# google-research/snap

Hardware: AMD Instinct MI355X
Metric: localization_scenes_per_sec (higher is better)
Workload: dtype f32 (tensors, accumulation, every non-GEMM op); conv / dense products on the bf16 matrix cores: operands split into 2 bf16 parts, 3 part products per MAC, ~2^-17 per product; 1 GPU; C2: 8 scenes/GPU, 4 StreetView views @512px + aerial, 128x128x60 voxel BEV @0.2m, ResNet-50 encoders, 10001 pose hypotheses; scenes_per_gpu=8, batches_in_flight=2, global_batch=8, parallelism=scene-sharded x1, no data-path collective, mode=inference forward (BEVLocalizer.apply, train=False)

## Files before the change

### include/snap_hip.h

```cpp
#ifndef SNAP_HIP_H_
#define SNAP_HIP_H_

#include <stddef.h>
#include <stdint.h>

#ifdef __cplusplus
extern "C" {
#endif

typedef enum SnapStatus {
  SNAP_OK = 0,
  SNAP_ERR_BAD_SHAPE = -1,
  SNAP_ERR_UNSUPPORTED = -2,
  SNAP_ERR_NULL = -3,
  SNAP_ERR_LAUNCH = -4,
  SNAP_ERR_WORKSPACE = -5
} SnapStatus;

#define SNAP_ABI_VERSION 29
int snap_abi_version(void);
const char* snap_status_string(int status);
const char* snap_build_arch(void);

enum { SNAP_PRO_NONE = 0, SNAP_PRO_AFFINE = 1, SNAP_PRO_GN_RELU = 2,
       SNAP_PRO_RELU_GN = 3, SNAP_PRO_RELU = 4 };
enum { SNAP_EPI_BIAS = 1, SNAP_EPI_RELU = 2, SNAP_EPI_RESIDUAL = 4,
       SNAP_EPI_UPSAMPLE2X_ADD = 8, SNAP_EPI_ROWMASK = 16,
       SNAP_EPI_GELU = 32  };

typedef struct SnapConvDesc {
  int32_t N, H, W, Cin, Cin_stride;
  int32_t KH, KW, stride, pad_t, pad_l;
  int32_t Ho, Wo, Cout, Cout_stride;
  int32_t prologue;
  int32_t epilogue;
  float in_scale, in_shift;
  int32_t tile_hint;
} SnapConvDesc;

int snap_conv2d_nhwc_f32(const SnapConvDesc* desc, const float* x, const float* w,
                         float* y, const float* gn_mu, const float* gn_sc,
                         const float* gn_beta, const float* bias,
                         const float* residual, const float* up_prev,
                         const uint8_t* row_mask, void* stream);

typedef struct SnapConvExtras {
  const int32_t* rows_in;
  const int32_t* rows_out;
  const int32_t* row_count;
  float* gn_partial;
  size_t gn_partial_bytes;
  int32_t gn_partial_relu;
  void* workspace;
  size_t workspace_bytes;
  const void* w_bf16;
  size_t w_bf16_bytes;
  int32_t w_split_parts;
  int32_t w_split_root;
  float* gn_partial2;
  size_t gn_partial2_bytes;
  int32_t gn_partial2_done;
  int32_t x_presplit;
  int32_t ps_tile;
  int32_t ps_res_init;
  int32_t bk_hint;
  int32_t tune_flags;
  int32_t gn_partial_rows;
  int32_t w_half;
  int32_t x_half;
  void* y_half;
  const float* gnb_x;
  const float* gnb_mu;
  const float* gnb_rstd;
  const float* gnb_gamma;
  const float* gnb_beta;
  int32_t gnb_mode;
} SnapConvExtras;
#define SNAP_TUNE_NO_HALO 1
#define SNAP_TUNE_NO_PLAIN 8
#define SNAP_TUNE_RS_NSPLIT_SHIFT 4
int32_t snap_conv2d_presplit_tile_rows(const SnapConvDesc* desc, int32_t ps_tile);
size_t snap_conv2d_presplit_gn_partial_bytes(const SnapConvDesc* desc, int32_t ps_tile);
size_t snap_conv2d_presplit_workspace_bytes(const SnapConvDesc* desc, int32_t ps_tile);
int32_t snap_conv2d_presplit_supported(const SnapConvDesc* desc);
int snap_gn_norm_split_f32(const float* y, const float* partial, int32_t N, int32_t HW, int32_t C,
                           int32_t groups, float eps, int32_t tile_rows, const float* gamma,
                           const float* beta, void* out, float* mu, float* sc, void* stream);
int snap_presplit_f32(const float* x, int64_t rows, int32_t C, void* out, void* stream);

int snap_conv2d_nhwc_ex_f32(const SnapConvDesc* desc, const float* x, const float* w,
                            float* y, const float* gn_mu, const float* gn_sc,
                            const float* gn_beta, const float* bias,
                            const float* residual, const float* up_prev,
                            const uint8_t* row_mask, const SnapConvExtras* extras,
                            void* stream);
size_t snap_conv2d_packed_weights_split_root_bytes(int32_t Cout, int32_t parts);
int snap_conv2d_pack_weights_split_root_bf16(const float* w , int32_t Cout,
                                             int32_t parts, void* out, size_t out_bytes,
                                             void* stream);
size_t snap_conv2d_packed_weights_bytes(int32_t taps, int32_t Cin, int32_t Cout);
int snap_conv2d_pack_weights_bf16(const float* w, int32_t taps, int32_t Cin, int32_t Cout,
                                  void* out, size_t out_bytes, void* stream);
int snap_conv2d_pack_weights_f16(const float* w, int32_t taps, int32_t Cin, int32_t Cout,
                                 void* out, size_t out_bytes, void* stream);
size_t snap_conv2d_packed_weights_split_bytes(int32_t taps, int32_t Cin, int32_t Cout,
                                              int32_t parts);
int snap_conv2d_pack_weights_split_bf16(const float* w, int32_t taps, int32_t Cin, int32_t Cout,
                                        int32_t parts, void* out, size_t out_bytes, void* stream);
typedef struct SnapPackItem {
  const float* w;
  void* out;
  int32_t taps, Cin, Cout, block_begin;
} SnapPackItem;
int32_t snap_conv2d_pack_weights_split_blocks(int32_t taps, int32_t Cin, int32_t Cout);
int32_t snap_conv2d_pack_weights_blocks(int32_t taps, int32_t Cin, int32_t Cout);
int snap_conv2d_pack_weights_multi_bf16(const SnapPackItem* items, int32_t n_items,
                                        int32_t total_blocks, void* stream);
int snap_conv2d_pack_weights_multi_f16(const SnapPackItem* items, int32_t n_items,
                                       int32_t total_blocks, void* stream);
int snap_conv2d_pack_weights_split_multi_bf16(const SnapPackItem* items, int32_t n_items,
                                              int32_t total_blocks, int32_t parts, void* stream);

int snap_interpolate_nd_f32(const float* array, const int32_t* size, int32_t n, int32_t D,
                            const uint8_t* valid_array, const float* points, int64_t K,
                            float* values, uint8_t* valid, void* stream);
int snap_expectation_nd_f32(const float* pdf, int64_t rows, const int32_t* size, int32_t n,
                            float* out, void* stream);
int snap_occupancy_ray_features_f32(const float* hits, const float* origins, const uint8_t* ray_mask,
                                    int64_t num_rays, int32_t num_samples, float margin, const float* points,
                                    int64_t num_points, int32_t B, const float* volume,
                                    const uint8_t* volume_valid, int32_t X, int32_t Y, int32_t Z, int32_t D,
                                    float cell_size, float* out_points, uint8_t* out_labels,
                                    uint8_t* out_ray_valid, float* features, uint8_t* valid, void* stream);
int32_t snap_occupancy_head_supported(int32_t D, int32_t h1, int32_t h2);
int snap_occupancy_head_f32(const float* hits, const float* origins, const uint8_t* ray_mask, int64_t num_rays,
                            int32_t num_samples, float margin, const float* points, int64_t num_points, int32_t B,
                            const float* volume, const uint8_t* volume_valid, int32_t X, int32_t Y, int32_t Z,
                            int32_t D, float cell_size, const float* w0, const float* b0, int32_t h1,
                            const float* w1, const float* b1, int32_t h2, const float* w_out,
                            const float* b_out, float* out_points, uint8_t* out_labels, uint8_t* out_ray_valid,
                            float* logits, uint8_t* valid, void* stream);
int32_t snap_occupancy_features_vjp_chunk(void);
size_t snap_occupancy_features_vjp_workspace_bytes(int64_t num_points, int32_t B, int32_t X, int32_t Y, int32_t Z,
                                                   int32_t D);
int snap_occupancy_ray_features_vjp_f32(const float* hits, const float* origins, const uint8_t* ray_mask,
                                        int64_t num_rays, int32_t num_samples, float margin, const float* points,
                                        int64_t num_points, int32_t B, int32_t X, int32_t Y, int32_t Z, int32_t D,
                                        float cell_size, const float* d_features, float* d_volume, void* workspace,
                                        size_t workspace_bytes, void* stream);

int snap_semantic_embed_f32(const uint8_t* rasters, int64_t M, int32_t N, const int32_t* idx_road,
                            int32_t nr, const int32_t* idx_other, int32_t no,
                            const float* table_road, const float* table_other, int32_t E,
                            float* out, void* stream);
int snap_semantic_onehot_f32(const uint8_t* rasters, int64_t M, int32_t N, const int32_t* idx_road,
                             int32_t nr, const int32_t* idx_other, int32_t no, float* onehot,
                             int32_t KP, void* stream);

int snap_layer_norm_f32(const float* x, const float* gamma, const float* beta, float* y,
                        int64_t M, int32_t C, float eps, void* stream);
int snap_attention_bf16_f32(const float* qkv, float* out, int32_t B, int32_t N, int32_t H,
                            int32_t D, float scale, void* stream);
int snap_layer_norm_bf16out_f32(const float* x, const float* gamma, const float* beta, void* y_bf16,
                                int64_t M, int32_t C, float eps, void* stream);
int snap_attention_bf16out_f32(const float* qkv, void* out_bf16, int32_t B, int32_t N, int32_t H,
                               int32_t D, float scale, void* stream);
int snap_attention_bf16io(const void* qkv_bf16, void* out_bf16, int32_t B, int32_t N, int32_t H, int32_t D,
                          float scale, void* stream);
int snap_attention_lse_bf16_f32(const float* qkv, float* out, float* lse, int32_t B, int32_t N,
                                int32_t H, int32_t D, float scale, void* stream);
int snap_attention_bwd_bf16_f32(const float* qkv, const float* out, const float* dout,
                                const float* lse, float* delta, float* dqkv, int32_t B, int32_t N,
                                int32_t H, int32_t D, float scale, void* stream);
size_t snap_layer_norm_bwd_workspace_bytes(int64_t M, int32_t C);
int snap_layer_norm_bwd_f32(const float* x, const float* dy, const float* gamma, float* dx,
                            float* dgamma, float* dbeta, int64_t M, int32_t C, float eps,
                            void* workspace, size_t workspace_bytes, void* stream);
int snap_gelu_f32(const float* x, float* y, int64_t n, void* stream);
int snap_gelu_bwd_f32(const float* x, const float* dy, float* dx, int64_t n, void* stream);

size_t snap_conv2d_workspace_bytes(const SnapConvDesc* desc);
size_t snap_conv2d_gn_partial_bytes(const SnapConvDesc* desc);
int32_t snap_conv2d_tile_rows(const SnapConvDesc* desc);
int32_t snap_conv2d_tile_rows_ex(const SnapConvDesc* desc, int32_t split_parts);
size_t snap_conv2d_gn_partial_bytes_ex(const SnapConvDesc* desc, int32_t split_parts);
size_t snap_conv2d_splitk_gn_partial_bytes(const SnapConvDesc* desc);
int32_t snap_conv2d_stationary_kind(const SnapConvDesc* desc, int32_t parts);

int32_t snap_conv2d_root_pool_supported(const SnapConvDesc* desc, int32_t parts);
int snap_conv2d_root_pool_f32(const SnapConvDesc* desc, const float* x, const void* w_bf16,
                              size_t w_bf16_bytes, int32_t parts, int32_t band_rows, float* y_pool,
                              void* stream);

int snap_group_norm_stats_from_partial_f32(const float* partial, const float* y, int32_t N,
                                           int32_t HW, int32_t C, int32_t groups, float eps,
                                           int32_t tile_rows, int32_t relu_first,
                                           const float* gamma, float* mu, float* sc, float* rstd,
                                           void* stream);

size_t snap_compact_rows_workspace_bytes(int64_t M);
int snap_compact_rows_u8(const uint8_t* mask, int64_t M, int32_t* index, int32_t* count,
                         void* workspace, size_t workspace_bytes, void* stream);
int snap_compact_rows_range_u8(const uint8_t* mask, int64_t M, int32_t lo, int32_t hi,
                               int32_t* index, int32_t* count, void* workspace,
                               size_t workspace_bytes, void* stream);

int snap_mlp2_pool_max_f32(const float* x, int64_t M, int32_t Cin, int32_t x_stride,
                           const int32_t* rows, const int32_t* row_count,
                           const void* w0_split, size_t w0_bytes, const float* b0, int32_t H,
                           const void* w1_split, size_t w1_bytes, const float* b1, int32_t D,
                           int32_t relu_in, int32_t x_split, int32_t Z, int64_t ncols,
                           float* plane, uint8_t* pvalid, void* stream);
int snap_mlp2_pool_max_classes_f32(const float* x, int64_t M, int32_t Cin, int32_t x_stride,
                                   const int32_t* rows, const int32_t* row_count,
                                   const int32_t* rows_z, const int32_t* row_count_z,
                                   int32_t zero_slab_lo, int32_t zero_slabs,
                                   const void* w0_split, size_t w0_bytes, const float* b0, int32_t H,
                                   const void* w1_split, size_t w1_bytes, const float* b1, int32_t D,
                                   int32_t relu_in, int32_t x_split, int32_t Z, int64_t ncols,
                                   float* plane, uint8_t* pvalid, void* stream);

int snap_mlp2_pool_max_gather_f32(const float* x, int64_t M, int32_t Cin, int32_t x_stride,
                                  const int32_t* rows, const int32_t* row_count,
                                  const int32_t* rows_g, const int32_t* row_count_g,
                                  const float* f_images, int64_t f_bytes, int32_t img_w,
                                  int32_t img_C, int32_t feature_dim, const uint32_t* tap_records,
                                  int32_t xcd_group, const void* w0_split, size_t w0_bytes,
                                  const float* b0, int32_t H, const void* w1_split, size_t w1_bytes,
                                  const float* b1, int32_t D, int32_t Z, int64_t ncols, float* plane,
                                  uint8_t* pvalid, void* stream);

int snap_fill_masked_rows_f32(float* y, const uint8_t* mask, int64_t M, int32_t C,
                              float value, void* stream);

int snap_pad_image_f32(const float* x, int32_t N, int32_t H, int32_t W, int32_t C, int32_t pad_h,
                       int32_t pad_w, int32_t pad_c, float* y, void* stream);

int snap_voxel_points_f32(const float* xy, int32_t xy_batched, const float* z, int32_t B, int32_t XY,
                          int32_t Z, float* out, void* stream);

int snap_weight_standardize_f32(const float* w, float* out, int32_t K,
                                int32_t Cout, float eps, void* stream);

typedef struct SnapWstdItem {
  const float* w;
  const float* dws;
  float* out;
  int32_t K, Cout, block_begin, reserved;
} SnapWstdItem;
int snap_weight_standardize_multi_f32(const SnapWstdItem* items, int32_t n_items,
                                      int32_t total_blocks, float eps, void* stream);
int snap_weight_standardize_bwd_multi_f32(const SnapWstdItem* items, int32_t n_items,
                                          int32_t total_blocks, float eps, void* stream);

size_t snap_group_norm_stats_workspace_bytes(int32_t N, int32_t HW, int32_t C,
                                             int32_t groups);
int snap_group_norm_stats_f32(const float* x, int32_t N, int32_t HW, int32_t C,
                              int32_t C_stride, int32_t groups, float eps,
                              int32_t relu_first, const float* gamma, float* mu,
                              float* sc, float* rstd ,
                              void* workspace, size_t workspace_bytes,
                              void* stream);

int snap_group_norm_apply_f32(const float* x, float* y, int32_t N, int32_t HW,
                              int32_t C, const float* mu, const float* sc,
                              const float* beta, int32_t mode, void* stream);

int snap_max_pool_3x3s2_f32(const float* x, float* y, int32_t N, int32_t H,
                            int32_t W, int32_t C, void* stream);

typedef struct SnapLiftDesc {
  int32_t B, V, h, w, C;
  int32_t feature_dim;
  int32_t num_bins;
  int32_t N;
  int32_t K;
  int32_t fisheye;
  int32_t out_stride;
  float depth_min, depth_max;
  float max_view_distance;
  int32_t weighted;
  int32_t use_variance;
  int32_t add_minmax;
  int32_t grid_y, grid_z;
  int32_t valid_rows_only;
  int32_t out_split;
  int32_t class_rows;
  int32_t tune_flags;
} SnapLiftDesc;

int snap_lift_pool_f32(const SnapLiftDesc* desc, const float* f_images,
                       const float* cam, const float* Rt, const float* points,
                       float* pooled, uint8_t* valid, void* stream);

int snap_lift_pool_records_f32(const SnapLiftDesc* desc, const float* f_images,
                               const float* cam, const float* Rt, const float* points,
                               float* pooled, uint8_t* valid, uint32_t* tap_records, void* stream);

int snap_lift_observations_f32(const SnapLiftDesc* desc, const float* f_images, const float* cam,
                               const float* Rt, const float* points, float* obs, float* obs_feat,
                               uint8_t* valid, void* stream);
int snap_lift_pool_observations_f32(const SnapLiftDesc* desc, const float* cam, const float* Rt,
                                    const float* points, const float* obs_feat, float* pooled,
                                    uint8_t* valid, void* stream);

int snap_project_points_f32(int32_t B, int32_t V, int32_t N, int32_t fisheye,
                            const float* cam, const float* Rt,
                            const float* points, float* p2d, uint8_t* vis,
                            float* depth, void* stream);

enum { SNAP_POOL_MAX = 0, SNAP_POOL_SUM = 1, SNAP_POOL_MEAN = 2 };

int snap_vertical_pool_f32(const float* vol, const uint8_t* vvalid, float* plane,
                           uint8_t* pvalid, int64_t M, int32_t Z, int32_t D,
                           int32_t pooling, void* stream);
int snap_vertical_pool_max_arg_f32(const float* vol, const uint8_t* vvalid, float* plane,
                                   uint8_t* pvalid, uint8_t* argz, uint8_t* ties, int64_t M,
                                   int32_t Z, int32_t D, void* stream);

int snap_plane_fuse_match_f32(const float* const* planes,
                              const uint8_t* const* valids, int32_t num_planes,
                              int64_t M, int32_t D, int32_t pooling, float* fused,
                              uint8_t* fvalid, const float* Wm, const float* bm,
                              int32_t Dm, int32_t normalize, float eps,
                              float* matching, void* stream);

#define SNAP_SIM_CHUNK 64

int snap_sim_softmax_f32(const float* fq, const float* fm, int32_t B, int32_t Nq,
                         int32_t XY, int32_t Dm, float scale,
                         int32_t clip_negative, const float* num_valid,
                         float* sim, float* chunk_stats, float* prob,
                         float* rowstats, void* stream);

size_t snap_sim_rowstats_bytes(int32_t B, int32_t Nq);

int snap_sim_softmax_weighted_f32(const float* fq, const float* fm, int32_t B, int32_t Nq,
                                  int32_t XY, int32_t Dm, float scale, int32_t clip_negative,
                                  const float* num_valid, const float* row_weight, float* sim,
                                  float* chunk_stats, float* prob, float* rowstats, void* stream);
size_t snap_sim_split_workspace_bytes(int32_t B, int32_t Nq, int32_t XY, int32_t Dm, int32_t parts);
int snap_sim_softmax_split_f32(const float* fq, const float* fm, int32_t B, int32_t Nq, int32_t XY,
                               int32_t Dm, float scale, int32_t clip_negative,
                               const float* num_valid, const float* row_weight, int32_t parts,
                               float* sim, float* chunk_stats, void* workspace,
                               size_t workspace_bytes, void* stream);
int snap_masked_softmax_rows_f32(const float* x, const uint8_t* mask, int32_t B, int32_t N,
                                 float* weights, float* cdf, void* stream);
int snap_confidence_head_f32(const float* features, const uint8_t* valid, const float* w,
                             const float* bias , int64_t M, int32_t D, float* out,
                             void* stream);
int snap_confidence_head_bwd_f32(const float* features, const uint8_t* valid, const float* w,
                                 const float* bias, const float* dconf, int64_t M, int32_t D,
                                 float* dfeatures, float* prod, float* dsv, void* stream);
int snap_sim_bwd_prepare_rows_f32(float* dsim, const float* sim, int32_t B, int32_t Nq, int32_t XY,
                                  int32_t clip_negative, const float* row_coef, float* rowdot,
                                  void* stream);
int snap_masked_softmax_rows_bwd_f32(const float* weights, const float* dweights, int32_t B,
                                     int32_t N, float* dx, void* stream);

int snap_ransac_sample_f32(const float* fq, const float* fm,
                           const float* chunk_stats, int32_t B, int32_t Nq,
                           int32_t X, int32_t Y, int32_t Dm, float scale,
                           int32_t clip_negative, int32_t S, uint64_t seed,
                           const float* uniforms, int32_t* corr, void* stream);

size_t snap_ransac_sample_workspace_bytes(int32_t B, int32_t Nq);
int snap_ransac_sample_sim_f32(const float* fq, const float* fm, const float* chunk_stats,
                               const float* row_cdf, const float* sim, const float* row_unscale,
                               int32_t B, int32_t Nq, int32_t X, int32_t Y, int32_t Dm, float scale,
                               int32_t clip_negative, int32_t S, uint64_t seed,
                               const float* uniforms, int32_t* corr, void* workspace,
                               size_t workspace_bytes, void* stream);
int snap_ransac_sample_rows_f32(const float* fq, const float* fm, const float* chunk_stats,
                                const float* row_cdf, int32_t B, int32_t Nq, int32_t X, int32_t Y,
                                int32_t Dm, float scale, int32_t clip_negative, int32_t S,
                                uint64_t seed, const float* uniforms, int32_t* corr,
                                void* workspace, size_t workspace_bytes, void* stream);
int snap_ransac_sample_ws_f32(const float* fq, const float* fm, const float* chunk_stats,
                              int32_t B, int32_t Nq, int32_t X, int32_t Y, int32_t Dm,
                              float scale, int32_t clip_negative, int32_t S, uint64_t seed,
                              const float* uniforms, int32_t* corr, void* workspace,
                              size_t workspace_bytes, void* stream);
// ... 321 lines not shown
```

### snap_amd/csrc/conv_common.h

```cpp
#ifndef SNAP_CSRC_CONV_COMMON_H_
#define SNAP_CSRC_CONV_COMMON_H_

#include <stdio.h>
#include <stdlib.h>

#include "common.h"

namespace snapconv {
struct ConvArgs {
  SnapConvDesc d;
  const float* x;
  const float* w;
  float* y;
  const float* gn_mu;
  const float* gn_sc;
  const float* gn_beta;
  const float* bias;
  const float* residual;
  const float* up_prev;
  const uint8_t* row_mask;
  const int32_t* rows_in;
  const int32_t* rows_out;
  const int32_t* row_count;
  float* kpartial;
  size_t kpartial_bytes;
  int ksplit;
  int slabs_per_split;
  int tiles_per_split;
  float* gn_partial;
  float* gn_partial2;
  int32_t* gn_partial2_done;
  int gn_relu;
  int gn_rows32;
  int gn_slabs;
  int M;
  int K;
  int ctiles;
  int nk;
  int ncol;
  int bk;
  int no_halo;
  int no_plain;
  int rs_nsplit;
  const void* w_bf16;
  int cin8;
  int half;
  const void* x_half;
  void* y_half;
  const void* x_ps;
  int ps_tile;
  int ps_res_init;
  int ps_parts;
  const float* gnb_x;
  const float* gnb_mu;
  const float* gnb_rstd;
  const float* gnb_gamma;
  const float* gnb_beta;
  int gnb_mode;
};

int launch_bf16(ConvArgs a, hipStream_t s);
int launch_split(ConvArgs a, int parts, hipStream_t s);
int launch_split_root(ConvArgs a, int parts, hipStream_t s);
int launch_ps(ConvArgs a, hipStream_t s);
int stationary_kind(const SnapConvDesc& d, int parts, bool row_lists);
int launch_rs(ConvArgs a, hipStream_t s);
int launch_bs(ConvArgs a, hipStream_t s);
int launch_root_ws(const ConvArgs& a, hipStream_t s);
struct PsTile { int bm, bn, nt; };
PsTile ps_choose_tile(int64_t M, int64_t N, int force);
int ps_ksplit(int64_t M, int Cout, int64_t nk, int bm, int bn, size_t kpartial_bytes);

}

namespace {
using snapconv::ConvArgs;

__device__ __attribute__((aligned(64))) const float kZeroChunk[16] = {0.f};

__device__ __forceinline__ float snap_gelu_tanh(float x) {
  const float u = 0.7978845608028654f * (x + 0.044715f * x * x * x);
  return x / (1.0f + __expf(-2.0f * u));
}

template <int BM, int BN, bool DUAL = false, int NT = 256, bool SKIP_RES = false, int OUTH = 0, bool GNB = false>
__device__ __forceinline__ void conv_epilogue(const ConvArgs& a,
                                              f32x16 (&acc)[BM / (NT / 4)][BN / 64],
                                              float* smem, int m0, int n0, int Meff, int row_t,
                                              int split) {
  constexpr int WR = NT / 128;
  constexpr int TM = BM / (32 * WR), TN = BN / 64;
  const SnapConvDesc& d = a.d;
  const int tid = threadIdx.x;
  const int lane = tid & 63;
  const int wid = tid >> 6;
  const int wr = wid >> 1, wc = wid & 1;
  const int l31 = lane & 31, lhi = lane >> 5;
  const int HoWo = d.Ho * d.Wo;
  const int epi = d.epilogue;
  const int Hp = d.Ho >> 1, Wp = d.Wo >> 1;
  constexpr int Q = BN / 4;
  constexpr int PER_THREAD = (32 * WR * Q) / NT;
  const bool want_stats = a.gn_partial != nullptr && a.ksplit == 1;
  const int n_first = m0 / HoWo;
  const int m_split = (n_first + 1) * HoWo;
  float gs1[2][4] = {{0.f, 0.f, 0.f, 0.f}, {0.f, 0.f, 0.f, 0.f}};
  float gs2[2][4] = {{0.f, 0.f, 0.f, 0.f}, {0.f, 0.f, 0.f, 0.f}};
  const bool want_relu_too = DUAL && want_stats;
  float hs1[2][4] = {{0.f, 0.f, 0.f, 0.f}, {0.f, 0.f, 0.f, 0.f}};
  float hs2[2][4] = {{0.f, 0.f, 0.f, 0.f}, {0.f, 0.f, 0.f, 0.f}};
  f32x4 vb_mu[2], vb_rs[2], vb_g = {0.f, 0.f, 0.f, 0.f}, vb_b = {0.f, 0.f, 0.f, 0.f};
  const bool gnb = GNB && want_stats && a.gnb_mode != 0;
  if constexpr (GNB) {
    vb_mu[0] = vb_mu[1] = vb_rs[0] = vb_rs[1] = vb_g;
    const int colq = n0 + 4 * (tid % Q);
    if (gnb && colq < d.Cout) {
      vb_g = *reinterpret_cast<const f32x4*>(a.gnb_gamma + colq);
      vb_b = *reinterpret_cast<const f32x4*>(a.gnb_beta + colq);
#pragma unroll
      for (int sl = 0; sl < 2; ++sl) {
        const int64_t so = (int64_t)min(n_first + sl, d.N - 1) * d.Cout + colq;
        vb_mu[sl] = *reinterpret_cast<const f32x4*>(a.gnb_mu + so);
        vb_rs[sl] = *reinterpret_cast<const f32x4*>(a.gnb_rstd + so);
      }
    }
  }
#pragma unroll
  for (int h = 0; h < TM; ++h) {
    if (h > 0) __syncthreads();
#pragma unroll
    for (int j = 0; j < TN; ++j)
#pragma unroll
      for (int r = 0; r < 16; ++r) {
        const int ri = (r & 3) + 8 * (r >> 2) + 4 * lhi;
        smem[(wr * 32 + ri) * BN + wc * (BN / 2) + j * 32 + l31] = acc[h][j][r];
      }
    __syncthreads();
#pragma unroll
    for (int it = 0; it < PER_THREAD; ++it) {
      const int idx = tid + NT * it;
      const int row = idx / Q, q = idx - row * Q;
      const int m = m0 + (row >> 5) * (BM / WR) + h * 32 + (row & 31);
      const int col = n0 + 4 * q;
      if (m >= Meff || col >= d.Cout) continue;
      f32x4 v = *reinterpret_cast<const f32x4*>(smem + row * BN + 4 * q);
      if (a.ksplit > 1) {
        *reinterpret_cast<f32x4*>(a.kpartial + ((int64_t)split * a.M + m) * d.Cout + col) = v;
        continue;
      }
      const int64_t o = (int64_t)(a.rows_out ? a.rows_out[m] : m) * d.Cout_stride + col;
      if (epi & SNAP_EPI_BIAS) {
        const f32x4 bb = *reinterpret_cast<const f32x4*>(a.bias + col);
#pragma unroll
        for (int e = 0; e < 4; ++e) v[e] += bb[e];
      }
      if (!SKIP_RES && (epi & SNAP_EPI_RESIDUAL)) {
        const f32x4 rr = *reinterpret_cast<const f32x4*>(a.residual + o);
#pragma unroll
        for (int e = 0; e < 4; ++e) v[e] += rr[e];
      }
      if (epi & SNAP_EPI_UPSAMPLE2X_ADD) {
        const int n = m / HoWo;
        const int rr = m - n * HoWo;
        const int ho = rr / d.Wo;
        const int wo = rr - ho * d.Wo;
        const float sh = (ho + 0.5f) * 0.5f - 0.5f;
        const float sw = (wo + 0.5f) * 0.5f - 0.5f;
        const float fh = floorf(sh), fw = floorf(sw);
        const float wh_hi = sh - fh, wh_lo = 1.f - wh_hi;
        const float ww_hi = sw - fw, ww_lo = 1.f - ww_hi;
        const int h0 = min(max((int)fh, 0), Hp - 1), h1 = min(max((int)fh + 1, 0), Hp - 1);
        const int w0 = min(max((int)fw, 0), Wp - 1), w1 = min(max((int)fw + 1, 0), Wp - 1);
        const int64_t base = (int64_t)n * Hp * Wp;
        const f32x4 p00 = *reinterpret_cast<const f32x4*>(
            a.up_prev + (base + (int64_t)h0 * Wp + w0) * d.Cout_stride + col);
        const f32x4 p01 = *reinterpret_cast<const f32x4*>(
            a.up_prev + (base + (int64_t)h0 * Wp + w1) * d.Cout_stride + col);
        const f32x4 p10 = *reinterpret_cast<const f32x4*>(
            a.up_prev + (base + (int64_t)h1 * Wp + w0) * d.Cout_stride + col);
        const f32x4 p11 = *reinterpret_cast<const f32x4*>(
            a.up_prev + (base + (int64_t)h1 * Wp + w1) * d.Cout_stride + col);
#pragma unroll
        for (int e = 0; e < 4; ++e) {
          const float c0 = p00[e] * wh_lo + p10[e] * wh_hi;
          const float c1 = p01[e] * wh_lo + p11[e] * wh_hi;
          v[e] += c0 * ww_lo + c1 * ww_hi;
        }
      }
      if (epi & SNAP_EPI_RELU) {
#pragma unroll
        for (int e = 0; e < 4; ++e) v[e] = snap_relu(v[e]);
      }
      if (epi & SNAP_EPI_GELU) {
#pragma unroll
        for (int e = 0; e < 4; ++e) v[e] = snap_gelu_tanh(v[e]);
      }
      if ((epi & SNAP_EPI_ROWMASK) && a.row_mask[m] == 0) v = f32x4{0.f, 0.f, 0.f, 0.f};
      if constexpr (OUTH == 0) {
        *reinterpret_cast<f32x4*>(a.y + o) = v;
      } else {
        if (a.y) *reinterpret_cast<f32x4*>(a.y + o) = v;
        store_half4<OUTH>(a.y_half, o, v);
      }
      if (GNB && gnb) {
        const int sl = m >= m_split ? 1 : 0;
        const f32x4 xv = *reinterpret_cast<const f32x4*>(a.gnb_x + (int64_t)m * d.Cout + col);
#pragma unroll
        for (int e = 0; e < 4; ++e) {
          float xh, dyp;
          if (a.gnb_mode == SNAP_PRO_GN_RELU) {
            xh = (xv[e] - vb_mu[sl][e]) * vb_rs[sl][e];
            dyp = (xh * vb_g[e] + vb_b[e] > 0.f) ? v[e] : 0.f;
          } else {
            xh = (fmaxf(xv[e], 0.f) - vb_mu[sl][e]) * vb_rs[sl][e];
            dyp = v[e];
          }
          gs1[sl][e] += dyp;
          gs2[sl][e] += dyp * xh;
        }
      } else if (want_stats) {
        const int sl = m >= m_split ? 1 : 0;
#pragma unroll
        for (int e = 0; e < 4; ++e) {
          const float t = a.gn_relu ? snap_relu(v[e]) : v[e];
          gs1[sl][e] += t;
          gs2[sl][e] += t * t;
          if constexpr (DUAL) {
            const float r = snap_relu(v[e]);
            hs1[sl][e] += r;
            hs2[sl][e] += r * r;
          }
        }
      }
    }
  }
  if (want_stats) {
    constexpr int RG = NT / Q;
    const int q = tid % Q, rg = tid / Q;
    for (int pass = 0; pass < (want_relu_too ? 2 : 1); ++pass) {
    float* const dst_partial = pass ? a.gn_partial2 : a.gn_partial;
    __syncthreads();
#pragma unroll
    for (int sl = 0; sl < 2; ++sl)
#pragma unroll
      for (int e = 0; e < 4; ++e) {
        smem[((rg * 2 + sl) * BN + 4 * q + e) * 2 + 0] = pass ? hs1[sl][e] : gs1[sl][e];
        smem[((rg * 2 + sl) * BN + 4 * q + e) * 2 + 1] = pass ? hs2[sl][e] : gs2[sl][e];
      }
    __syncthreads();
    for (int i = tid; i < 2 * BN; i += NT) {
      const int sl = i / BN, c = i - sl * BN;
      const int col = n0 + c;
      const int n = n_first + sl;
      const bool live = col < d.Cout && n < d.N && (sl == 0 || (m0 + BM > m_split && m_split < Meff));
      if (!live) continue;
      float t1 = 0.f, t2 = 0.f;
#pragma unroll
      for (int r = 0; r < RG; ++r) {
        t1 += smem[((r * 2 + sl) * BN + c) * 2 + 0];
        t2 += smem[((r * 2 + sl) * BN + c) * 2 + 1];
      }
      const int slab = row_t - (int)(((int64_t)n * HoWo) / BM);
      float* o = dst_partial + (((int64_t)n * a.gn_slabs + slab) * d.Cout + col) * 2;
      o[0] = t1;
      o[1] = t2;
    }
    }
  }
}

__global__ __launch_bounds__(256) void splitk_reduce_kernel(
    const float* __restrict__ partial, int S, int64_t M, int Cout, int Cout_stride, int epi,
    const float* __restrict__ bias, const float* __restrict__ residual,
    const uint8_t* __restrict__ row_mask, float* __restrict__ y) {
  const int Q = Cout >> 2;
  const int64_t i = (int64_t)blockIdx.x * blockDim.x + threadIdx.x;
  if (i >= M * Q) return;
  const int64_t m = i / Q;
  const int col = 4 * (int)(i - m * Q);
  f32x4 v = *reinterpret_cast<const f32x4*>(partial + m * Cout + col);
  int s = 1;
  for (; s + 3 < S; s += 4) {
    f32x4 t[4];
#pragma unroll
    for (int u = 0; u < 4; ++u)
      t[u] = *reinterpret_cast<const f32x4*>(partial + ((int64_t)(s + u) * M + m) * Cout + col);
#pragma unroll
    for (int u = 0; u < 4; ++u)
#pragma unroll
      for (int e = 0; e < 4; ++e) v[e] += t[u][e];
  }
  for (; s < S; ++s) {
    const f32x4 t = *reinterpret_cast<const f32x4*>(partial + ((int64_t)s * M + m) * Cout + col);
#pragma unroll
    for (int e = 0; e < 4; ++e) v[e] += t[e];
  }
  const int64_t o = m * Cout_stride + col;
  if (epi & SNAP_EPI_BIAS) {
    const f32x4 bb = *reinterpret_cast<const f32x4*>(bias + col);
#pragma unroll
    for (int e = 0; e < 4; ++e) v[e] += bb[e];
  }
  if (epi & SNAP_EPI_RESIDUAL) {
    const f32x4 rr = *reinterpret_cast<const f32x4*>(residual + o);
#pragma unroll
    for (int e = 0; e < 4; ++e) v[e] += rr[e];
  }
  if (epi & SNAP_EPI_RELU) {
#pragma unroll
    for (int e = 0; e < 4; ++e) v[e] = snap_relu(v[e]);
  }
  if (epi & SNAP_EPI_GELU) {
#pragma unroll
    for (int e = 0; e < 4; ++e) v[e] = snap_gelu_tanh(v[e]);
  }
  if ((epi & SNAP_EPI_ROWMASK) && row_mask[m] == 0) v = f32x4{0.f, 0.f, 0.f, 0.f};
  *reinterpret_cast<f32x4*>(y + o) = v;
}

__global__ __launch_bounds__(256) void splitk_reduce_stats_kernel(
    const float* __restrict__ partial, int S, int64_t M, int Cout, int epi,
    const float* __restrict__ bias, const float* __restrict__ residual,
    const uint8_t* __restrict__ row_mask, float* __restrict__ y, int HoWo, int N, int gn_slabs,
    int gn_relu, float* __restrict__ gn_partial) {
  __shared__ float red[256 * 16];
  const int Q = Cout >> 2;
  const int QW = Q < 256 ? Q : 256;
  const int PW = 256 / QW;
  const int tq = threadIdx.x % QW, tp = threadIdx.x / QW;
  const int64_t m0 = (int64_t)blockIdx.x * 32;
  const int n_first = (int)(m0 / HoWo);
  const int64_t m_split = (int64_t)(n_first + 1) * HoWo;
  for (int q0 = 0; q0 < Q; q0 += QW) {
    const int q = q0 + tq;
    const int col = 4 * q;
    float s1[2][4] = {{0.f, 0.f, 0.f, 0.f}, {0.f, 0.f, 0.f, 0.f}};
    float s2[2][4] = {{0.f, 0.f, 0.f, 0.f}, {0.f, 0.f, 0.f, 0.f}};
    if (q < Q && tp < PW) {
      constexpr int RB = 8;
      for (int r0 = tp; r0 < 32; r0 += RB * PW) {
        f32x4 v[RB];
        bool ok[RB];
#pragma unroll
        for (int k = 0; k < RB; ++k) {
          const int64_t m = m0 + r0 + k * PW;
          ok[k] = r0 + k * PW < 32 && m < M;
          v[k] = *reinterpret_cast<const f32x4*>(partial + (ok[k] ? m : m0) * Cout + col);
        }
        for (int sp = 1; sp < S; ++sp) {
          f32x4 t[RB];
#pragma unroll
          for (int k = 0; k < RB; ++k)
            t[k] = *reinterpret_cast<const f32x4*>(partial + ((int64_t)sp * M + (ok[k] ? m0 + r0 + k * PW : m0)) * Cout + col);
#pragma unroll
          for (int k = 0; k < RB; ++k)
#pragma unroll
            for (int e = 0; e < 4; ++e) v[k][e] += t[k][e];
        }
        f32x4 bb = {0.f, 0.f, 0.f, 0.f};
        if (epi & SNAP_EPI_BIAS) bb = *reinterpret_cast<const f32x4*>(bias + col);
        f32x4 rr[RB];
        if (epi & SNAP_EPI_RESIDUAL) {
#pragma unroll
          for (int k = 0; k < RB; ++k)
            rr[k] = *reinterpret_cast<const f32x4*>(residual + (ok[k] ? m0 + r0 + k * PW : m0) * Cout + col);
        }
#pragma unroll
        for (int k = 0; k < RB; ++k) {
          if (!ok[k]) continue;
          const int64_t m = m0 + r0 + k * PW;
          const int64_t o = m * Cout + col;
          if (epi & SNAP_EPI_BIAS) {
#pragma unroll
            for (int e = 0; e < 4; ++e) v[k][e] += bb[e];
          }
          if (epi & SNAP_EPI_RESIDUAL) {
#pragma unroll
            for (int e = 0; e < 4; ++e) v[k][e] += rr[k][e];
          }
          if (epi & SNAP_EPI_RELU) {
#pragma unroll
            for (int e = 0; e < 4; ++e) v[k][e] = snap_relu(v[k][e]);
          }
          if (epi & SNAP_EPI_GELU) {
#pragma unroll
            for (int e = 0; e < 4; ++e) v[k][e] = snap_gelu_tanh(v[k][e]);
          }
          if ((epi & SNAP_EPI_ROWMASK) && row_mask[m] == 0) v[k] = f32x4{0.f, 0.f, 0.f, 0.f};
          *reinterpret_cast<f32x4*>(y + o) = v[k];
          const int sl = m >= m_split ? 1 : 0;
#pragma unroll
          for (int e = 0; e < 4; ++e) {
            const float t = gn_relu ? snap_relu(v[k][e]) : v[k][e];
            s1[sl][e] += t;
            s2[sl][e] += t * t;
          }
        }
      }
    }
    __syncthreads();
#pragma unroll
    for (int sl = 0; sl < 2; ++sl)
#pragma unroll
      for (int e = 0; e < 4; ++e) {
        red[threadIdx.x * 16 + sl * 8 + e] = s1[sl][e];
        red[threadIdx.x * 16 + sl * 8 + 4 + e] = s2[sl][e];
      }
    __syncthreads();
    if (tp == 0 && q < Q) {
#pragma unroll
      for (int sl = 0; sl < 2; ++sl) {
        const int n = n_first + sl;
        const bool live = n < N && (sl == 0 || (m0 + 32 > m_split && m_split < M));
        if (!live) continue;
        const int slab = (int)(blockIdx.x - (((int64_t)n * HoWo) >> 5));
        float* o = gn_partial + (((int64_t)n * gn_slabs + slab) * Cout + col) * 2;
#pragma unroll
        for (int e = 0; e < 4; ++e) {
          float t1 = 0.f, t2 = 0.f;
          for (int pp = 0; pp < PW; ++pp) {
            t1 += red[(pp * QW + tq) * 16 + sl * 8 + e];
            t2 += red[(pp * QW + tq) * 16 + sl * 8 + 4 + e];
          }
          o[2 * e] = t1;
          o[2 * e + 1] = t2;
        }
      }
    }
  }
}

inline int launch_splitk_reduce(const ConvArgs& a, hipStream_t s) {
  if (a.gn_partial) {
    if (!a.gn_rows32 || (a.d.Cout & 3) || (256 % ((a.d.Cout >> 2) < 256 ? (a.d.Cout >> 2) : 256)) != 0)
      return SNAP_ERR_UNSUPPORTED;
    hipLaunchKernelGGL(splitk_reduce_stats_kernel, dim3((unsigned)snap_cdiv((int64_t)a.M, 32)), dim3(256), 0, s,
                       (const float*)a.kpartial, a.ksplit, (int64_t)a.M, a.d.Cout, a.d.epilogue, a.bias,
                       a.residual, a.row_mask, a.y, a.d.Ho * a.d.Wo, a.d.N, (a.d.Ho * a.d.Wo) / 32 + 2,
                       a.gn_relu, a.gn_partial);
  } else {
    const int64_t total4 = (int64_t)a.M * (a.d.Cout / 4);
    hipLaunchKernelGGL(splitk_reduce_kernel, dim3((unsigned)snap_cdiv(total4, 256)), dim3(256), 0, s,
                       (const float*)a.kpartial, a.ksplit, (int64_t)a.M, a.d.Cout, a.d.Cout_stride,
                       a.d.epilogue, a.bias, a.residual, a.row_mask, a.y);
  }
  SNAP_CHECK_LAUNCH();
  return SNAP_OK;
}

constexpr int64_t splitk_max_tiles() { return 384; }
constexpr int splitk_target() { return 768; }

struct TileChoice { int bm, bn; };
inline int hint_tile(int h) { return h % 1000000; }
inline int hint_mode(int h) { return h / 1000000; }
inline int64_t desc_k(const SnapConvDesc& d) { return (int64_t)d.KH * d.KW * d.Cin; }
inline TileChoice choose_tile(int64_t M, int64_t N, int forced, int64_t K) {
  forced = hint_tile(forced);
  const int64_t kMin = 512;
  const bool n_wide_ok = N > 64 && !(N % 128 != 0 && N % 128 <= 64);
  if (forced != 128128 && forced != 128064 && forced != 64128 && forced != 64064) forced = 0;
  if (forced == 128128 || (!forced && n_wide_ok && snap_cdiv(M, 128) * snap_cdiv(N, 128) >= kMin))
    return {128, 128};
  if (!forced && n_wide_ok && K >= 2304 && M >= 128) return {128, 128};
  const int64_t t64128 = snap_cdiv(M, 64) * snap_cdiv(N, 128);
  if (!forced && n_wide_ok && N >= 512 && K >= 1024 && t64128 >= kMin) return {64, 128};
  if (forced == 128064 || (!forced && snap_cdiv(M, 128) * snap_cdiv(N, 64) >= kMin)) return {128, 64};
  if (forced == 64128 || (!forced && n_wide_ok && N >= 512 && t64128 >= kMin)) return {64, 128};
  if (!forced && n_wide_ok && K >= 1024 && t64128 >= 256) return {64, 128};
  return {64, 64};
}

}

#endif
```

### snap_amd/csrc/conv_igemm.hip

```cpp
#include "conv_common.h"

namespace {

template <int BM, int BN, bool VEC, int PRO, int BK, bool DMA = false>
__device__ __forceinline__ void conv_igemm_body(const ConvArgs& a) {
  constexpr int AS = BM + 2;
  constexpr int TM = BM / 64;
  constexpr int TN = BN / 64;
  constexpr int QPR = BK / 4;
  constexpr int RPP = 256 / QPR;
  constexpr int AROWS = BM / RPP;
  constexpr int SRPP = 256 / BK;
  constexpr int AELEMS = BM / SRPP;
  constexpr int BQ = BN / 4;
  constexpr int BROWS_PER_PASS = 256 / BQ;
  constexpr int BPASS = BK / BROWS_PER_PASS;

  constexpr int kDmaStages = 3;
  constexpr int kSlabFloats = DMA ? kDmaStages * (BK * BM + BK * BN) : 2 * BK * AS + 2 * BK * BN;
  constexpr int kStageFloats = 64 * BN;
  constexpr int kSmemFloats = kSlabFloats > kStageFloats ? kSlabFloats : kStageFloats;
  __shared__ __attribute__((aligned(16))) float smem[kSmemFloats];
  float* const As0 = smem;
  float* const Bs0 = smem + 2 * BK * AS;
// ... 304 lines not shown
#pragma unroll
        for (int j = 0; j < TN; ++j)
          bv[nx][j] = bs[(2 * (kk + 1) + lhi) * BN + wc * (BN / 2) + j * 32 + l31];
      }
#pragma unroll
      for (int i = 0; i < TM; ++i)
#pragma unroll
        for (int j = 0; j < TN; ++j)
          acc[i][j] =
              __builtin_amdgcn_mfma_f32_32x32x2f32(av[cu][i], bv[cu][j], acc[i][j], 0, 0, 0);
    }
    __builtin_amdgcn_sched_group_barrier(0x100, TM + TN, 0);
#pragma unroll
    for (int kk = 0; kk < BK / 2; ++kk) {
      if (kk + 1 < BK / 2) __builtin_amdgcn_sched_group_barrier(0x100, TM + TN, 0);
      __builtin_amdgcn_sched_group_barrier(0x008, TM * TN, 0);
    }
    if (more) store_slab(cur ^ 1);
    __syncthreads();
  }

  }

  conv_epilogue<BM, BN>(a, acc, smem, m0, n0, Meff, row_t, split);
}

template <int BM, int BN, bool VEC, int PRO, int BK>
__global__ __launch_bounds__(256) void conv_igemm_kernel(const ConvArgs a) {
  conv_igemm_body<BM, BN, VEC, PRO, BK>(a);
}
template <int BM, int BN, bool VEC, int PRO, int BK>
__global__ __launch_bounds__(256) __attribute__((amdgpu_waves_per_eu(4, 4)))
void conv_igemm_kernel_occ4(const ConvArgs a) {
  conv_igemm_body<BM, BN, VEC, PRO, BK>(a);
}
template <int BM, int BN, int PRO>
__global__ __launch_bounds__(256) void conv_igemm_kernel_dma(const ConvArgs a) {
  conv_igemm_body<BM, BN, true, PRO, 16, true>(a);
}

template <int BM, int BN, bool VEC, int PRO, int BK>
int launch(ConvArgs a, hipStream_t s) {
  if (VEC) {
    a.ctiles = (a.d.Cin + BK - 1) / BK;
    a.nk = a.d.KH * a.d.KW * a.ctiles;
  } else {
    a.ctiles = 0;
    a.nk = (a.K + BK - 1) / BK;
  }
  const int64_t nrow = snap_cdiv(a.M, BM);
  a.ncol = (int)snap_cdiv(a.d.Cout, BN);
  a.gn_slabs = (a.d.Ho * a.d.Wo) / BM + 2;
  int64_t nblocks = snap_cdiv(nrow, 8) * 8 * a.ncol;
  if (nblocks > 0x7fffffffLL) return SNAP_ERR_BAD_SHAPE;
  a.ksplit = 1;
  a.tiles_per_split = (int)nblocks;
  a.slabs_per_split = a.nk;
  const int64_t tiles = nrow * a.ncol;
  const int target = splitk_target();
  if (a.kpartial && target > 0 && tiles <= splitk_max_tiles() && a.nk >= 16 && !a.rows_in &&
      !a.rows_out && !a.row_count && !a.gn_partial &&
      !(a.d.epilogue & SNAP_EPI_UPSAMPLE2X_ADD)) {
    int64_t S = (target + tiles - 1) / tiles;
    S = S < a.nk / 8 ? S : a.nk / 8;
    const int64_t fit = (int64_t)(a.kpartial_bytes / ((size_t)a.M * a.d.Cout * sizeof(float)));
    S = S < fit ? S : fit;
    if (S >= 2) {
      a.slabs_per_split = (int)((a.nk + S - 1) / S);
      a.ksplit = (a.nk + a.slabs_per_split - 1) / a.slabs_per_split;
      nblocks *= a.ksplit;
    }
  }
  constexpr bool kGn = PRO == SNAP_PRO_GN_RELU || PRO == SNAP_PRO_RELU_GN;
  constexpr bool kDmaOk = VEC && BK == 16 && (PRO == SNAP_PRO_NONE || PRO == SNAP_PRO_RELU);
  bool launched = false;
  if constexpr (kDmaOk) {
    if (a.d.Cin % 4 == 0) {
      hipLaunchKernelGGL((conv_igemm_kernel_dma<BM, BN, PRO>), dim3((unsigned)nblocks), dim3(256), 0,
                         s, a);
      launched = true;
    }
  }
  if (launched) {
  } else if constexpr (!kGn && BK == 16 && (VEC || BM * BN < 128 * 128)) {
    hipLaunchKernelGGL((conv_igemm_kernel_occ4<BM, BN, VEC, PRO, BK>), dim3((unsigned)nblocks),
                       dim3(256), 0, s, a);
  } else {
    hipLaunchKernelGGL((conv_igemm_kernel<BM, BN, VEC, PRO, BK>), dim3((unsigned)nblocks),
                       dim3(256), 0, s, a);
  }
  SNAP_CHECK_LAUNCH();
  if (a.ksplit > 1) {
    const int64_t total4 = (int64_t)a.M * (a.d.Cout / 4);
    hipLaunchKernelGGL(splitk_reduce_kernel, dim3((unsigned)snap_cdiv(total4, 256)), dim3(256), 0, s,
                       (const float*)a.kpartial, a.ksplit, (int64_t)a.M, a.d.Cout, a.d.Cout_stride,
                       a.d.epilogue, a.bias, a.residual, a.row_mask, a.y);
    SNAP_CHECK_LAUNCH();
  }
  return SNAP_OK;
}

template <int BM, int BN, bool VEC, int BK>
int launch_pro(const ConvArgs& a, hipStream_t s) {
  switch (a.d.prologue) {
    case SNAP_PRO_NONE: return launch<BM, BN, VEC, SNAP_PRO_NONE, BK>(a, s);
    case SNAP_PRO_AFFINE: return launch<BM, BN, VEC, SNAP_PRO_AFFINE, BK>(a, s);
    case SNAP_PRO_GN_RELU:
      if constexpr (VEC) return launch<BM, BN, VEC, SNAP_PRO_GN_RELU, BK>(a, s);
      return SNAP_ERR_UNSUPPORTED;
    case SNAP_PRO_RELU_GN:
      if constexpr (VEC) return launch<BM, BN, VEC, SNAP_PRO_RELU_GN, BK>(a, s);
      return SNAP_ERR_UNSUPPORTED;
    case SNAP_PRO_RELU: return launch<BM, BN, VEC, SNAP_PRO_RELU, BK>(a, s);
    default: return SNAP_ERR_UNSUPPORTED;
  }
}


template <bool VEC>
int launch_tile(const ConvArgs& a, hipStream_t s) {
  const TileChoice t = choose_tile(a.M, a.d.Cout, a.d.tile_hint, desc_k(a.d));
  const bool deep = VEC && a.bk == 32 && a.d.Cin >= 32;
  if (t.bm == 128 && t.bn == 128) {
    if constexpr (VEC) {
      if (deep) return launch_pro<128, 128, VEC, 32>(a, s);
    }
    return launch_pro<128, 128, VEC, 16>(a, s);
  }
  if (t.bm == 128) {
    if constexpr (VEC) {
      if (deep) return launch_pro<128, 64, VEC, 32>(a, s);
    }
    return launch_pro<128, 64, VEC, 16>(a, s);
  }
  if (t.bn == 128) return launch_pro<64, 128, VEC, 16>(a, s);
  return launch_pro<64, 64, VEC, 16>(a, s);
}

}

extern "C" int snap_conv2d_nhwc_f32(const SnapConvDesc* desc, const float* x,
                                    const float* w, float* y, const float* gn_mu,
                                    const float* gn_sc, const float* gn_beta,
                                    const float* bias, const float* residual,
                                    const float* up_prev, const uint8_t* row_mask,
                                    void* stream) {
  return snap_conv2d_nhwc_ex_f32(desc, x, w, y, gn_mu, gn_sc, gn_beta, bias, residual, up_prev,
                                 row_mask, nullptr, stream);
}

extern "C" int32_t snap_conv2d_tile_rows_ex(const SnapConvDesc* desc, int32_t split_parts) {
  if (!desc) return 0;
  const int kind = snapconv::stationary_kind(*desc, split_parts, false);
  if (kind == 3) return -(desc->H * ((desc->W + 29) / 30));
  if (kind == 2) return 32;
  return choose_tile((int64_t)desc->N * desc->Ho * desc->Wo, desc->Cout, desc->tile_hint, desc_k(*desc)).bm;
}

extern "C" size_t snap_conv2d_gn_partial_bytes_ex(const SnapConvDesc* desc, int32_t split_parts) {
  if (!desc) return 0;
  const SnapConvDesc& d = *desc;
  const int64_t HoWo = (int64_t)d.Ho * d.Wo;
  const int bm = snap_conv2d_tile_rows_ex(desc, split_parts);
  if (bm < 0) return (size_t)d.N * (size_t)(-bm) * d.Cout * 2 * sizeof(float);
  if (HoWo < bm) return 0;
  return (size_t)d.N * (HoWo / bm + 2) * d.Cout * 2 * sizeof(float);
}

extern "C" size_t snap_conv2d_gn_partial_bytes(const SnapConvDesc* desc) {
  return snap_conv2d_gn_partial_bytes_ex(desc, 0);
}

extern "C" size_t snap_conv2d_splitk_gn_partial_bytes(const SnapConvDesc* desc) {
  if (!desc || snap_conv2d_workspace_bytes(desc) == 0) return 0;
  const SnapConvDesc& d = *desc;
  const int64_t HoWo = (int64_t)d.Ho * d.Wo;
  const int q = d.Cout >> 2;
  if (HoWo < 32 || (d.Cout & 3) || d.Cout_stride != d.Cout || 256 % (q < 256 ? q : 256) != 0) return 0;
  return (size_t)d.N * (HoWo / 32 + 2) * d.Cout * 2 * sizeof(float);
}

extern "C" size_t snap_conv2d_workspace_bytes(const SnapConvDesc* desc) {
  if (!desc) return 0;
  const SnapConvDesc& d = *desc;
  const int64_t M = (int64_t)d.N * d.Ho * d.Wo;
  const TileChoice t = choose_tile(M, d.Cout, d.tile_hint, desc_k(d));
  const int64_t tiles = snap_cdiv(M, t.bm) * snap_cdiv((int64_t)d.Cout, t.bn);
  const int target = splitk_target();
  const int64_t nk = (int64_t)d.KH * d.KW * ((d.Cin + 15) / 16);
  if (target <= 0 || tiles > splitk_max_tiles() || nk < 16 || (d.epilogue & SNAP_EPI_UPSAMPLE2X_ADD)) return 0;
  int64_t S = (target + tiles - 1) / tiles;
  S = S < nk / 8 ? S : nk / 8;
  if (S < 2) return 0;
  return (size_t)S * M * d.Cout * sizeof(float);
}

extern "C" int32_t snap_conv2d_tile_rows(const SnapConvDesc* desc) {
  return snap_conv2d_tile_rows_ex(desc, 0);
}

extern "C" int32_t snap_conv2d_stationary_kind(const SnapConvDesc* desc, int32_t parts) {
  if (!desc) return 0;
  return snapconv::stationary_kind(*desc, parts, false);
}

extern "C" int32_t snap_conv2d_presplit_tile_rows(const SnapConvDesc* desc, int32_t ps_tile) {
  if (!desc) return 0;
  return snapconv::ps_choose_tile((int64_t)desc->N * desc->Ho * desc->Wo, desc->Cout, ps_tile).bm;
}

extern "C" size_t snap_conv2d_presplit_gn_partial_bytes(const SnapConvDesc* desc, int32_t ps_tile) {
  if (!desc) return 0;
  const SnapConvDesc& d = *desc;
  const int64_t HoWo = (int64_t)d.Ho * d.Wo;
  const snapconv::PsTile t = snapconv::ps_choose_tile((int64_t)d.N * HoWo, d.Cout, ps_tile);
  if (HoWo < t.bm) return 0;
  return (size_t)d.N * (HoWo / t.bm + 2) * d.Cout * 2 * sizeof(float);
}

extern "C" size_t snap_conv2d_presplit_workspace_bytes(const SnapConvDesc* desc, int32_t ps_tile) {
  if (!desc) return 0;
  const SnapConvDesc& d = *desc;
  if (d.Cin % 16 != 0 || (d.epilogue & SNAP_EPI_UPSAMPLE2X_ADD)) return 0;
  const int64_t M = (int64_t)d.N * d.Ho * d.Wo;
  const snapconv::PsTile t = snapconv::ps_choose_tile(M, d.Cout, ps_tile);
  const int64_t nk = (int64_t)d.KH * d.KW * (d.Cin / 16);
  const int S = snapconv::ps_ksplit(M, d.Cout, nk, t.bm, t.bn, (size_t)-1);
  return S >= 2 ? (size_t)S * M * d.Cout * sizeof(float) : 0;
}

extern "C" int snap_conv2d_nhwc_ex_f32(const SnapConvDesc* desc, const float* x,
                                       const float* w, float* y, const float* gn_mu,
                                       const float* gn_sc, const float* gn_beta,
                                       const float* bias, const float* residual,
                                       const float* up_prev, const uint8_t* row_mask,
                                       const SnapConvExtras* ex, void* stream) {
  if (!desc || !x || !w || (!y && !(ex && ex->y_half))) return SNAP_ERR_NULL;
  const int32_t* rows_in = ex ? ex->rows_in : nullptr;
  const int32_t* rows_out = ex ? ex->rows_out : nullptr;
  const int32_t* row_count = ex ? ex->row_count : nullptr;
  float* gn_partial = ex ? ex->gn_partial : nullptr;
  if ((rows_in || rows_out) &&
      (desc->epilogue & (SNAP_EPI_RESIDUAL | SNAP_EPI_UPSAMPLE2X_ADD | SNAP_EPI_ROWMASK)))
    return SNAP_ERR_UNSUPPORTED;
  if (ex && (ex->tune_flags & 2)) return SNAP_ERR_UNSUPPORTED;
  const bool presplit = ex && ex->x_presplit;
  const bool split_vec = ex && ex->w_bf16 && !ex->w_split_root && !rows_in && !rows_out && !row_count;
  const bool rows32 = gn_partial && ex->gn_partial_rows == 32;
  if (gn_partial && ex->gn_partial_rows != 0 && ex->gn_partial_rows != 32) return SNAP_ERR_BAD_SHAPE;
  if (rows32 && (presplit || !split_vec || ex->w_split_parts == 1 || !ex->workspace || ex->gn_partial2 ||
                 ex->y_half || ex->gnb_mode))
    return SNAP_ERR_UNSUPPORTED;
  const size_t gn_need = !gn_partial ? 0
                         : rows32    ? snap_conv2d_splitk_gn_partial_bytes(desc)
                         : presplit  ? snap_conv2d_presplit_gn_partial_bytes(desc, ex->ps_tile)
                                     : snap_conv2d_gn_partial_bytes_ex(desc, split_vec ? ex->w_split_parts : 0);
  if (gn_partial) {
    if (rows_in || rows_out || row_count) return SNAP_ERR_UNSUPPORTED;
    if (desc->Cout_stride != desc->Cout) return SNAP_ERR_UNSUPPORTED;
    if (ex->gn_partial_bytes < gn_need || gn_need == 0) return SNAP_ERR_WORKSPACE;
  }
  const SnapConvDesc& d = *desc;
  if (d.N <= 0 || d.H <= 0 || d.W <= 0 || d.Cin <= 0 || d.Cout <= 0 || d.KH <= 0 ||
      d.KW <= 0 || d.stride <= 0 || d.Ho <= 0 || d.Wo <= 0)
    return SNAP_ERR_BAD_SHAPE;
  if (d.Cin_stride < d.Cin || d.Cout_stride < d.Cout) return SNAP_ERR_BAD_SHAPE;
  if (d.Cout % 4 != 0 || d.Cout_stride % 4 != 0) return SNAP_ERR_BAD_SHAPE;
  if ((reinterpret_cast<uintptr_t>(y) & 15) || (reinterpret_cast<uintptr_t>(w) & 15) ||
      (reinterpret_cast<uintptr_t>(bias) & 15) || (reinterpret_cast<uintptr_t>(residual) & 15) ||
      (reinterpret_cast<uintptr_t>(up_prev) & 15))
    return SNAP_ERR_BAD_SHAPE;
  if ((int64_t)d.N * d.Ho * d.Wo > 0x7fffffffLL) return SNAP_ERR_BAD_SHAPE;
  const bool gn = d.prologue == SNAP_PRO_GN_RELU || d.prologue == SNAP_PRO_RELU_GN;
  if (d.prologue < 0 || d.prologue > SNAP_PRO_RELU) return SNAP_ERR_UNSUPPORTED;
  if (gn && (!gn_mu || !gn_sc || !gn_beta)) return SNAP_ERR_NULL;
  if ((d.epilogue & SNAP_EPI_BIAS) && !bias) return SNAP_ERR_NULL;
  if ((d.epilogue & SNAP_EPI_RESIDUAL) && !residual) return SNAP_ERR_NULL;
  if ((d.epilogue & SNAP_EPI_ROWMASK) && !row_mask) return SNAP_ERR_NULL;
  if (d.epilogue & SNAP_EPI_UPSAMPLE2X_ADD) {
    if (!up_prev) return SNAP_ERR_NULL;
    if ((d.Ho & 1) || (d.Wo & 1)) return SNAP_ERR_BAD_SHAPE;
  }
  ConvArgs a;
  a.d = d;
  a.x = x; a.w = w; a.y = y;
  a.gn_mu = gn_mu; a.gn_sc = gn_sc; a.gn_beta = gn_beta;
  a.bias = bias; a.residual = residual; a.up_prev = up_prev; a.row_mask = row_mask;
  a.rows_in = rows_in; a.rows_out = rows_out; a.row_count = row_count;
  a.gn_partial = gn_partial;
  a.gn_relu = ex ? ex->gn_partial_relu : 0;
  a.gn_rows32 = rows32 ? 1 : 0;
  a.gn_partial2 = nullptr;
  a.gn_partial2_done = nullptr;
  if (gn_partial && ex->gn_partial2) {
    if (a.gn_relu || ex->gn_partial2_bytes < gn_need) return SNAP_ERR_WORKSPACE;
    a.gn_partial2 = ex->gn_partial2;
    a.gn_partial2_done = const_cast<int32_t*>(&ex->gn_partial2_done);
    *a.gn_partial2_done = 0;
  }
  a.kpartial = ex ? static_cast<float*>(ex->workspace) : nullptr;
  a.kpartial_bytes = ex ? ex->workspace_bytes : 0;
  if (reinterpret_cast<uintptr_t>(a.kpartial) & 15) a.kpartial = nullptr;
  a.ksplit = 1; a.slabs_per_split = 0; a.tiles_per_split = 0;
  a.gn_slabs = 0;
  a.M = d.N * d.Ho * d.Wo;
  a.K = d.KH * d.KW * d.Cin;
  const bool vec = (d.Cin_stride % 4 == 0) && (d.Cin >= 4) &&
                   ((reinterpret_cast<uintptr_t>(x) & 15) == 0) &&
                   (!gn || (d.Cin % 4 == 0));
  a.ctiles = 0;
  a.nk = 0;
  a.bk = (ex && ex->bk_hint == 32) ? 32 : 16;
  a.no_halo = (ex && (ex->tune_flags & SNAP_TUNE_NO_HALO)) ? 1 : 0;
  a.rs_nsplit = ex ? (ex->tune_flags >> SNAP_TUNE_RS_NSPLIT_SHIFT) & 15 : 0;
  a.no_plain = (ex && (ex->tune_flags & SNAP_TUNE_NO_PLAIN)) ? 1 : 0;
  hipStream_t s = static_cast<hipStream_t>(stream);
  a.w_bf16 = ex ? ex->w_bf16 : nullptr;
  a.half = (ex && ex->w_half) ? 1 : 0;
  if (a.half && (ex->w_split_parts != 0 || presplit || ex->w_split_root)) return SNAP_ERR_UNSUPPORTED;
  a.x_half = nullptr;
  a.y_half = nullptr;
  const bool ps1 = presplit && ex->w_split_parts == 1;
  if (ex && ex->y_half) {
    if (!a.w_bf16 || (ex->w_split_parts != 0 && !ps1) || (presplit && !ps1) || ex->w_split_root || gn_partial ||
        (d.epilogue & SNAP_EPI_UPSAMPLE2X_ADD) || d.Cout_stride % 4 != 0 ||
        (reinterpret_cast<uintptr_t>(ex->y_half) & 7))
      return SNAP_ERR_UNSUPPORTED;
    a.y_half = ex->y_half;
    a.kpartial = nullptr;
  }
  a.gnb_x = a.gnb_mu = a.gnb_rstd = a.gnb_gamma = a.gnb_beta = nullptr;
  a.gnb_mode = 0;
  if (ex && ex->gnb_mode) {
    if ((ex->gnb_mode != SNAP_PRO_GN_RELU && ex->gnb_mode != SNAP_PRO_RELU_GN) || !ex->x_half || !gn_partial ||
        ex->gn_partial_rows != 0 || ex->gn_partial2 || ex->gn_partial_relu || ex->workspace ||
        (d.epilogue & ~(SNAP_EPI_RESIDUAL | SNAP_EPI_BIAS)))
      return SNAP_ERR_UNSUPPORTED;
    if (!ex->gnb_x || !ex->gnb_mu || !ex->gnb_rstd || !ex->gnb_gamma || !ex->gnb_beta) return SNAP_ERR_NULL;
    if ((reinterpret_cast<uintptr_t>(ex->gnb_x) | reinterpret_cast<uintptr_t>(ex->gnb_mu) |
         reinterpret_cast<uintptr_t>(ex->gnb_rstd) | reinterpret_cast<uintptr_t>(ex->gnb_gamma) |
         reinterpret_cast<uintptr_t>(ex->gnb_beta)) & 15)
      return SNAP_ERR_BAD_SHAPE;
    a.gnb_x = ex->gnb_x; a.gnb_mu = ex->gnb_mu; a.gnb_rstd = ex->gnb_rstd;
    a.gnb_gamma = ex->gnb_gamma; a.gnb_beta = ex->gnb_beta;
    a.gnb_mode = ex->gnb_mode;
  }
  a.cin8 = (d.Cin + 7) / 8 * 8;
  a.x_ps = nullptr;
  a.ps_tile = 0;
  a.ps_res_init = 0;
  a.ps_parts = 2;
  if (ex && ex->x_half) {
    if (!a.w_bf16 || ex->w_split_parts != 0 || presplit || ex->w_split_root || d.prologue != SNAP_PRO_NONE ||
        rows_in || d.Cin_stride % 8 != 0 || d.Cin % 8 != 0 || ex->y_half)
      return SNAP_ERR_UNSUPPORTED;
    if (ex->w_bf16_bytes < snap_conv2d_packed_weights_bytes(d.KH * d.KW, d.Cin, d.Cout)) return SNAP_ERR_WORKSPACE;
    if ((reinterpret_cast<uintptr_t>(a.w_bf16) | reinterpret_cast<uintptr_t>(x)) & 15) return SNAP_ERR_BAD_SHAPE;
    a.x_half = x;
    a.x = nullptr;
    return snapconv::launch_bf16(a, s);
  }
  if (presplit) {
    if (!a.w_bf16 || (ex->w_split_parts != 2 && ex->w_split_parts != 1) || ex->w_split_root) return SNAP_ERR_UNSUPPORTED;
    if (ps1 && d.Cin_stride != d.Cin) return SNAP_ERR_UNSUPPORTED;
    a.ps_parts = ex->w_split_parts;
    const size_t need = snap_conv2d_packed_weights_split_bytes(d.KH * d.KW, d.Cin, d.Cout, ex->w_split_parts);
    if (need == 0) return SNAP_ERR_UNSUPPORTED;
    if (ex->w_bf16_bytes < need) return SNAP_ERR_WORKSPACE;
    if ((reinterpret_cast<uintptr_t>(a.w_bf16) | reinterpret_cast<uintptr_t>(x)) & 15) return SNAP_ERR_BAD_SHAPE;
    a.x_ps = x;
    a.x = nullptr;
    a.ps_tile = ex->ps_tile;
    a.ps_res_init = ex->ps_res_init;
    a.cin8 = d.Cin;
    return snapconv::launch_ps(a, s);
  }
  if (a.w_bf16 && ex->w_split_root) {
    const int parts = ex->w_split_parts;
    if (ex->w_bf16_bytes < snap_conv2d_packed_weights_split_root_bytes(d.Cout, parts) ||
        snap_conv2d_packed_weights_split_root_bytes(d.Cout, parts) == 0)
      return SNAP_ERR_WORKSPACE;
    if ((reinterpret_cast<uintptr_t>(a.w_bf16) | reinterpret_cast<uintptr_t>(x)) & 15) return SNAP_ERR_BAD_SHAPE;
    a.cin8 = 16;
    return snapconv::launch_split_root(a, parts, s);
  }
  if (a.w_bf16 && vec) {
    const int parts = ex->w_split_parts;
    if (parts < 0 || parts == 1 || parts > 3) return SNAP_ERR_UNSUPPORTED;
    const size_t need = parts ? snap_conv2d_packed_weights_split_bytes(d.KH * d.KW, d.Cin, d.Cout, parts)
                              : snap_conv2d_packed_weights_bytes(d.KH * d.KW, d.Cin, d.Cout);
    if (need == 0) return SNAP_ERR_UNSUPPORTED;
    if (ex->w_bf16_bytes < need) return SNAP_ERR_WORKSPACE;
    if (parts) a.cin8 = (d.Cin + 15) / 16 * 16;
    if (reinterpret_cast<uintptr_t>(a.w_bf16) & 15) return SNAP_ERR_BAD_SHAPE;
    return parts ? snapconv::launch_split(a, parts, s) : snapconv::launch_bf16(a, s);
  }
  return vec ? launch_tile<true>(a, s) : launch_tile<false>(a, s);
}
```

### snap_amd/csrc/conv_split.hip

```cpp
#include "conv_common.h"

namespace {


template <int BM, int BN, int PRO, int NS, bool GNT, bool TAIL, bool ROOT = false, bool DUAL = false, bool PLAIN = false>
__device__ __forceinline__ void conv_split_body(const ConvArgs& a) {
  constexpr int BK = 16;
  constexpr int TM = BM / 64;
  constexpr int TN = BN / 64;
  constexpr int QPR = BK / 4;
  constexpr int RPP = 256 / QPR;
  constexpr int AROWS = BM / RPP;
  constexpr int A_PART = BM * 32;
  constexpr int B_PART = BN * 32;
  constexpr int A_ST = NS * A_PART;
  constexpr int B_ST = NS * B_PART;
  constexpr int BSLOTS = NS * BN * 2;
  constexpr int BPIECES = (BSLOTS + 255) / 256;
  constexpr int kSlabBytes = 2 * (A_ST + B_ST);
  constexpr int kStageBytes = 64 * BN * 4;
  constexpr int kSmemBytes = kSlabBytes > kStageBytes ? kSlabBytes : kStageBytes;
  constexpr bool need_gn = (PRO == SNAP_PRO_GN_RELU || PRO == SNAP_PRO_RELU_GN);
  constexpr bool gn_tab = need_gn && GNT;
  constexpr int kGnRing = 320;
  __shared__ __attribute__((aligned(16))) float smem[(kSmemBytes + (gn_tab ? 3 * kGnRing : 0)) / 4];
  char* const Ab = reinterpret_cast<char*>(smem);
  char* const Bb = Ab + 2 * A_ST;
  char* const Gt = Ab + kSmemBytes;

  const SnapConvDesc& d = a.d;
  const int tid = threadIdx.x;
  const int lane = tid & 63;
  const int wid = tid >> 6;
  const int wr = wid >> 1, wc = wid & 1;
  const int ncol = a.ncol;
  const int split = a.ksplit > 1 ? blockIdx.x / a.tiles_per_split : 0;
  const int bid = a.ksplit > 1 ? blockIdx.x - split * a.tiles_per_split : blockIdx.x;
  const int xcd = bid & 7;
  const int seq = bid >> 3;
  const int col_t = seq % ncol;
  const int row_t = (seq / ncol) * 8 + xcd;
  const int Meff = a.row_count ? min(*a.row_count, a.M) : a.M;
  if (row_t * BM >= Meff) return;
  const int m0 = row_t * BM;
  const int n0 = col_t * BN;
  const int HoWo = d.Ho * d.Wo;
  const int n_first = m0 / HoWo;
  const int m_split = (n_first + 1) * HoWo;

  int r_hb[AROWS], r_wb[AROWS];
  bool r_ok[AROWS];
  const float* r_px[AROWS];
  int64_t r_gn[AROWS];
  int r_slot[AROWS];
  int r_voff[AROWS];
#pragma unroll
  for (int i = 0; i < AROWS; ++i) {
    const int row = (tid / QPR) + RPP * i;
    const int m = m0 + row;
    r_ok[i] = m < Meff;
    int mm = r_ok[i] ? m : (PLAIN ? Meff - 1 : 0);
    if (a.rows_in) mm = a.rows_in[mm];
    const int n = mm / HoWo;
    const int r = mm - n * HoWo;
    const int ho = r / d.Wo;
    const int wo = r - ho * d.Wo;
    r_hb[i] = ho * d.stride - d.pad_t;
    r_wb[i] = wo * d.stride - d.pad_l;
    r_px[i] = a.x + (((int64_t)n * d.H + r_hb[i]) * d.W + r_wb[i]) * d.Cin_stride;
    r_gn[i] = (int64_t)n * d.Cin;
    r_slot[i] = (PLAIN ? mm : m) >= m_split ? 1 : 0;
    if constexpr (PLAIN) r_voff[i] = (int)(((int64_t)(mm - m0) * d.Cin_stride + 4 * (tid % QPR)) * 4);
  }
  const int akq = tid % QPR;
  const int64_t x_left = ((int64_t)(Meff - m0) * d.Cin_stride) * 4;
  const __amdgpu_buffer_rsrc_t rs_x = __builtin_amdgcn_make_buffer_rsrc(
      const_cast<float*>(a.x) + (PLAIN ? (int64_t)m0 * d.Cin_stride : 0), 0,
      (int)(x_left < 0x7ff00000LL ? x_left : 0x7ff00000LL), 0x00020000);

  f32x16 acc[TM][TN];
#pragma unroll
  for (int i = 0; i < TM; ++i)
#pragma unroll
    for (int j = 0; j < TN; ++j)
#pragma unroll
      for (int r = 0; r < 16; ++r) acc[i][j][r] = 0.f;

  f32x4 xa[AROWS], xmu[AROWS], xsc[AROWS], xbeta;
  bool xin[AROWS];
  int cur_c = 0;

  const int taps = d.KH * d.KW;
  const int kt_begin = a.ksplit > 1 ? split * a.slabs_per_split : 0;
  const int kt_end = a.ksplit > 1 ? min(a.nk, kt_begin + a.slabs_per_split) : a.nk;
  int kpos = 0, ct = 0, kh = 0, kw = 0;
  if (kt_begin > 0) {
    kpos = kt_begin / a.ctiles;
    ct = kt_begin - kpos * a.ctiles;
    kh = kpos / d.KW;
    kw = kpos - kh * d.KW;
  }
  const float* tap_px[AROWS];
  bool tap_in[AROWS];
  auto set_tap = [&]() {
    const int64_t delta = ((int64_t)kh * d.W + (ROOT ? 4 * kw : kw)) * d.Cin_stride;
#pragma unroll
    for (int i = 0; i < AROWS; ++i) {
      const int hi = r_hb[i] + kh, wi = r_wb[i] + (ROOT ? 4 * kw + (tid % QPR) : kw);
      tap_in[i] = r_ok[i] && hi >= 0 && hi < d.H && wi >= 0 && wi < d.W;
      tap_px[i] = r_px[i] + delta;
    }
  };
  set_tap();

  auto load_a = [&]() {
    if constexpr (PLAIN) {
      static_assert(!PLAIN || (GNT || !need_gn), "PLAIN takes the table variant of the GroupNorm prologue");
#pragma unroll
      for (int i = 0; i < AROWS; ++i) {
        const u32x4 r = __builtin_amdgcn_raw_buffer_load_b128(rs_x, r_voff[i], ct * (BK * 4), 0);
        __builtin_memcpy(&xa[i], &r, 16);
      }
      return;
    }
    const int c = ct * BK + 4 * akq;
    cur_c = c;
    const bool cvalid = ROOT || c < d.Cin;
    if constexpr (need_gn && !gn_tab)
      xbeta = *reinterpret_cast<const f32x4*>(a.gn_beta + (cvalid ? c : 0));
#pragma unroll
    for (int i = 0; i < AROWS; ++i) {
      const bool inb = tap_in[i] && cvalid;
      xin[i] = inb;
      const float* px = inb ? tap_px[i] + c : a.x;
      xa[i] = *reinterpret_cast<const f32x4*>(px);
      if constexpr (need_gn && !gn_tab) {
        const int64_t so = inb ? r_gn[i] + c : (int64_t)0;
        xmu[i] = *reinterpret_cast<const f32x4*>(a.gn_mu + so);
        xsc[i] = *reinterpret_cast<const f32x4*>(a.gn_sc + so);
      }
    }
  };
  const char* const wt = static_cast<const char*>(a.w_bf16);
  const int64_t col_tile_bytes = (int64_t)taps * a.ctiles * (NS * 4096);
  const char* bsrc[BPIECES];
#pragma unroll
  for (int p = 0; p < BPIECES; ++p) {
    const int slot = tid + 256 * p;
    const int part = slot / (2 * BN);
    const int rem = slot - part * (2 * BN);
    const int gcol = n0 + (rem >> 1);
    bsrc[p] = wt + (gcol >> 7) * col_tile_bytes + (int64_t)kt_begin * (NS * 4096) +
              (part < NS ? part : 0) * 4096 + (gcol & 127) * 32 + (rem & 1) * 16;
  }
  auto issue_b = [&](int buf) {
#pragma unroll
    for (int p = 0; p < BPIECES; ++p) {
      const int slot = tid + 256 * p;
      if (BSLOTS % 256 != 0 && slot >= BSLOTS) break;
      lds_dma16(bsrc[p], Bb + buf * B_ST + 16 * slot);
      bsrc[p] += NS * 4096;
    }
  };
  const int n_second = min(n_first + 1, d.N - 1);
  auto issue_gn = [&](int ring, int ctile) {
    if constexpr (gn_tab) {
      if (tid < 20) {
        const int seg = tid >> 2;
        const int c = ctile * BK + 4 * (tid & 3);
        const float* base = seg == 4 ? a.gn_beta
                                     : ((seg & 1) ? a.gn_sc : a.gn_mu) +
                                           (int64_t)(seg >= 2 ? n_second : n_first) * d.Cin;
        const void* src = c < d.Cin ? static_cast<const void*>(base + c)
                                    : static_cast<const void*>(kZeroChunk);
        lds_dma16(src, Gt + ring * kGnRing + 16 * tid);
      }
    }
  };
  auto advance = [&]() {
    if (++ct == a.ctiles) {
      ct = 0;
      ++kpos;
      if (++kw == d.KW) { kw = 0; ++kh; }
      set_tap();
    }
  };
  auto store_a = [&](int buf, int ring) {
    const float* const tb = reinterpret_cast<const float*>(Gt + ring * kGnRing);
    if constexpr (gn_tab) xbeta = *reinterpret_cast<const f32x4*>(tb + 64 + 4 * akq);
#pragma unroll
    for (int i = 0; i < AROWS; ++i) {
      const int row = (tid / QPR) + RPP * i;
      f32x4 v = xa[i];
      if constexpr (gn_tab) {
        xmu[i] = *reinterpret_cast<const f32x4*>(tb + r_slot[i] * 32 + 4 * akq);
        xsc[i] = *reinterpret_cast<const f32x4*>(tb + r_slot[i] * 32 + 16 + 4 * akq);
      }
#pragma unroll
      for (int e = 0; e < 4; ++e) {
        float pv;
        if constexpr (need_gn)
          pv = apply_pro<PRO>(v[e], xmu[i][e], xsc[i][e], xbeta[e], d.in_scale, d.in_shift);
        else
          pv = apply_pro<PRO>(v[e], 0.f, 0.f, 0.f, d.in_scale, d.in_shift);
        if constexpr (PLAIN)
          v[e] = pv;
        else if constexpr (TAIL)
          v[e] = (xin[i] && (cur_c + e < d.Cin)) ? pv : 0.f;
        else
          v[e] = xin[i] ? pv : 0.f;
      }
      u32x2 parts[NS];
      split_bf16<NS>(v, parts);
      const int oct = (akq >> 1) ^ ((row >> 3) & 1);
      char* dst = Ab + buf * A_ST + row * 32 + oct * 16 + (akq & 1) * 8;
#pragma unroll
      for (int p = 0; p < NS; ++p) *reinterpret_cast<u32x2*>(dst + p * A_PART) = parts[p];
    }
  };

  const int l31 = lane & 31, lhi = lane >> 5;
  int g_ct = ct;
  auto next_gct = [&]() { if (++g_ct == a.ctiles) g_ct = 0; };
  int ring_cur = 0;
  if (kt_begin < kt_end) {
    if constexpr (gn_tab) {
      issue_gn(0, g_ct); next_gct();
      issue_gn(1, g_ct); next_gct();
    }
    load_a();
    issue_b(0);
    advance();
    if constexpr (gn_tab) {
      wait_vm<0>();
      __syncthreads();
    }
    store_a(0, 0);
    wait_vm<0>();
    __syncthreads();
  }
  for (int kt = kt_begin; kt < kt_end; ++kt) {
    const int cur = (kt - kt_begin) & 1;
    const bool more = kt + 1 < kt_end;
    const int ring_next = ring_cur == 2 ? 0 : ring_cur + 1;
    if (more) {
      load_a();
      issue_b(cur ^ 1);
      advance();
      if constexpr (gn_tab) {
        if (kt + 2 < kt_end) { issue_gn(ring_next == 2 ? 0 : ring_next + 1, g_ct); next_gct(); }
      }
    }
    const char* as = Ab + cur * A_ST;
    const char* bs = Bb + cur * B_ST;
    bf16x8 av[TM][NS], bv[TN][NS];
#pragma unroll
    for (int i = 0; i < TM; ++i)
      load_frag<NS>(as + frag_offset(wr * (BM / 2) + i * 32 + l31, lhi), A_PART, av[i]);
#pragma unroll
    for (int j = 0; j < TN; ++j)
      load_frag<NS>(bs + frag_offset(wc * (BN / 2) + j * 32 + l31, lhi), B_PART, bv[j]);
    split_product<NS>(acc, av, bv);
    if (more) store_a(cur ^ 1, ring_next);
    ring_cur = ring_next;
    wait_vm<0>();
    __syncthreads();
  }

  conv_epilogue<BM, BN, DUAL>(a, acc, smem, m0, n0, Meff, row_t, split);
}

template <int BN, int PRO, int NS, int HPMAX>
__device__ __forceinline__ void conv3x3_halo_body(const ConvArgs& a) {
  constexpr int BM = 128, BK = 16;
  constexpr int TM = 2, TN = BN / 64;
  constexpr int NPER = (HPMAX * 4 + 255) / 256;
  constexpr int H_PART = HPMAX * 32;
  constexpr int H_ST = NS * H_PART;
  constexpr int B_PART = BN * 32;
  constexpr int B_ST = NS * B_PART;
  constexpr int BSLOTS = NS * BN * 2;
  constexpr int BPIECES = (BSLOTS + 255) / 256;
  constexpr int kSlabBytes = 2 * (H_ST + B_ST);
  constexpr int kStageBytes = 64 * BN * 4;
  constexpr int kSmemBytes = kSlabBytes > kStageBytes ? kSlabBytes : kStageBytes;
  constexpr bool need_gn = (PRO == SNAP_PRO_GN_RELU || PRO == SNAP_PRO_RELU_GN);
  constexpr int kGnRing = 320;
  __shared__ __attribute__((aligned(16))) float smem[(kSmemBytes + (need_gn ? 2 * kGnRing : 0)) / 4];
  char* const Hb = reinterpret_cast<char*>(smem);
  char* const Bb = Hb + 2 * H_ST;
  char* const Gt = Hb + kSmemBytes;

  const SnapConvDesc& d = a.d;
  const int tid = threadIdx.x;
  const int lane = tid & 63;
  const int wid = tid >> 6;
  const int wr = wid >> 1, wc = wid & 1;
  const int l31 = lane & 31, lhi = lane >> 5;
  const int ncol = a.ncol;
  const int split = a.ksplit > 1 ? blockIdx.x / a.tiles_per_split : 0;
  const int bid = a.ksplit > 1 ? blockIdx.x - split * a.tiles_per_split : blockIdx.x;
  const int xcd = bid & 7;
  const int seq = bid >> 3;
  const int col_t = seq % ncol;
  const int row_t = (seq / ncol) * 8 + xcd;
  const int Meff = a.M;
  if (row_t * BM >= Meff) return;
  const int m0 = row_t * BM;
  const int n0 = col_t * BN;
  const int W = d.W, HW = d.H * d.W;
  const int n_first = m0 / HW;
  const int m_split = (n_first + 1) * HW;
  const int n_second = min(n_first + 1, d.N - 1);
  const int halo0 = m0 - W - 1;
  const int HP = BM + 2 * W + 2;

  int tapmask[TM];
#pragma unroll
  for (int i = 0; i < TM; ++i) {
    const int m = m0 + wr * 64 + i * 32 + l31;
    int mk = 0;
    if (m < Meff) {
      const int r = m % HW;
      const int y = r / W, x = r - y * W;
#pragma unroll
      for (int t = 0; t < 9; ++t) {
        const int yy = y + t / 3 - 1, xx = x + t % 3 - 1;
        if (yy >= 0 && yy < d.H && xx >= 0 && xx < W) mk |= 1 << t;
      }
    }
    tapmask[i] = mk;
  }

  const int Mtot = d.N * HW;
  auto halo_ok_row = [&](int hp) {
    const int mp = halo0 + hp;
    return hp < HP && mp >= 0 && mp < Mtot;
  };
  f32x4 xa[NPER];
  auto load_halo = [&](int ct) {
#pragma unroll
    for (int j = 0; j < NPER; ++j) {
      const int f = tid + 256 * j;
      const int hp = f >> 2;
      const bool ok = halo_ok_row(hp);
      const float* px = a.x + ((int64_t)(ok ? halo0 + hp : 0) * d.Cin_stride + 4 * (f & 3) + ct * BK);
      xa[j] = *reinterpret_cast<const f32x4*>(ok ? px : a.x);
    }
  };
  auto issue_gn = [&](int ring, int ct) {
    if constexpr (need_gn) {
      if (tid < 20) {
        const int seg = tid >> 2;
        const int c = ct * BK + 4 * (tid & 3);
        const float* base = seg == 4 ? a.gn_beta
                                     : ((seg & 1) ? a.gn_sc : a.gn_mu) +
                                           (int64_t)(seg >= 2 ? n_second : n_first) * d.Cin;
        lds_dma16(base + c, Gt + ring * kGnRing + 16 * tid);
      }
    }
  };
  auto store_halo = [&](int buf, int ring) {
    const float* const tb = reinterpret_cast<const float*>(Gt + ring * kGnRing);
#pragma unroll
    for (int j = 0; j < NPER; ++j) {
      const int f = tid + 256 * j;
      const int hp = f >> 2, q = f & 3;
      if (NPER * 256 > HPMAX * 4 && hp >= HPMAX) continue;
      f32x4 v = xa[j];
      f32x4 mu = {0.f, 0.f, 0.f, 0.f}, sc = mu, be = mu;
      const bool ok = halo_ok_row(hp);
      if constexpr (need_gn) {
        const int slot = halo0 + hp >= m_split ? 1 : 0;
        mu = *reinterpret_cast<const f32x4*>(tb + slot * 32 + 4 * q);
        sc = *reinterpret_cast<const f32x4*>(tb + slot * 32 + 16 + 4 * q);
        be = *reinterpret_cast<const f32x4*>(tb + 64 + 4 * q);
      }
#pragma unroll
      for (int e = 0; e < 4; ++e) {
        const float pv = apply_pro<PRO>(v[e], mu[e], sc[e], be[e], d.in_scale, d.in_shift);
        v[e] = ok ? pv : 0.f;
      }
      u32x2 parts[NS];
      split_bf16<NS>(v, parts);
      const int oct = (q >> 1) ^ ((hp >> 3) & 1);
      char* dst = Hb + buf * H_ST + hp * 32 + oct * 16 + (q & 1) * 8;
#pragma unroll
      for (int p = 0; p < NS; ++p) *reinterpret_cast<u32x2*>(dst + p * H_PART) = parts[p];
    }
  };

  const char* const wt = static_cast<const char*>(a.w_bf16);
  const int ctiles = a.ctiles;
  const int64_t col_tile_bytes = (int64_t)9 * ctiles * (NS * 4096);
  const char* bbase[BPIECES];
#pragma unroll
  for (int p = 0; p < BPIECES; ++p) {
    const int slot = tid + 256 * p;
    const int part = slot / (2 * BN);
    const int rem = slot - part * (2 * BN);
    const int gcol = n0 + (rem >> 1);
    bbase[p] = wt + (gcol >> 7) * col_tile_bytes + (part < NS ? part : 0) * 4096 + (gcol & 127) * 32 +
               (rem & 1) * 16;
  }
  auto issue_b = [&](int buf, int ct, int t) {
    const int64_t off = ((int64_t)t * ctiles + ct) * (NS * 4096);
#pragma unroll
    for (int p = 0; p < BPIECES; ++p) {
      const int slot = tid + 256 * p;
      if (BSLOTS % 256 != 0 && slot >= BSLOTS) break;
      lds_dma16(bbase[p] + off, Bb + buf * B_ST + 16 * slot);
    }
  };

  f32x16 acc[TM][TN];
#pragma unroll
  for (int i = 0; i < TM; ++i)
#pragma unroll
    for (int j = 0; j < TN; ++j)
#pragma unroll
      for (int r = 0; r < 16; ++r) acc[i][j][r] = 0.f;

  const int ct_begin = a.ksplit > 1 ? split * a.slabs_per_split : 0;
  const int ct_end = a.ksplit > 1 ? min(ctiles, ct_begin + a.slabs_per_split) : ctiles;
  issue_gn(0, ct_begin);
  load_halo(ct_begin);
  issue_b(0, ct_begin, 0);
  if constexpr (need_gn) {
    wait_vm<0>();
    __syncthreads();
  }
  store_halo(0, 0);
  wait_vm<0>();
  __syncthreads();

  int bcur = 0;
  for (int ct = ct_begin; ct < ct_end; ++ct) {
    const int hb = (ct - ct_begin) & 1;
    const bool more_ct = ct + 1 < ct_end;
#pragma unroll 1
    for (int t = 0; t < 9; ++t) {
      const bool last = !more_ct && t == 8;
      const bool fetch = t == 0 && more_ct;
      if (fetch) issue_gn(hb ^ 1, ct + 1);
      if (!last) issue_b(bcur ^ 1, t == 8 ? ct + 1 : ct, t == 8 ? 0 : t + 1);
      if (fetch) {
        asm volatile("" ::: "memory");
        load_halo(ct + 1);
        asm volatile("" ::: "memory");
      }
      const int kh = t / 3, kw = t - 3 * kh;
      const int toff = kh * W + kw;
      const char* hs = Hb + hb * H_ST;
      const char* bs = Bb + bcur * B_ST;
      bf16x8 av[TM][NS], bv[TN][NS];
#pragma unroll
      for (int i = 0; i < TM; ++i) {
        const int h = wr * 64 + i * 32 + l31 + toff;
        const char* p0 = hs + frag_offset(h, lhi);
        const bool in = (tapmask[i] >> t) & 1;
#pragma unroll
        for (int p = 0; p < NS; ++p) {
          u32x4 raw = *reinterpret_cast<const u32x4*>(p0 + p * H_PART);
          if (!in) raw = u32x4{0u, 0u, 0u, 0u};
          __builtin_memcpy(&av[i][p], &raw, 16);
        }
      }
#pragma unroll
      for (int j = 0; j < TN; ++j)
        load_frag<NS>(bs + frag_offset(wc * (BN / 2) + j * 32 + l31, lhi), B_PART, bv[j]);
      split_product<NS>(acc, av, bv);
      if (t == 2 && more_ct) store_halo(hb ^ 1, hb ^ 1);
      if (fetch)
        wait_vm<NPER>();
      else
        wait_vm<0>();
      asm volatile("s_waitcnt lgkmcnt(0)\n\ts_barrier" ::: "memory");
      bcur ^= 1;
    }
  }
  conv_epilogue<BM, BN>(a, acc, smem, m0, n0, Meff, row_t, split);
}

template <int BN, int PRO, int NS, int HPMAX>
__global__ __launch_bounds__(256, NS == 2 ? 3 : 2) void conv3x3_halo_kernel(const ConvArgs a) {
  conv3x3_halo_body<BN, PRO, NS, HPMAX>(a);
}

inline bool halo_ok(const ConvArgs& a) {
  const bool on = !a.no_halo;
  const SnapConvDesc& d = a.d;
  const int hp = 128 + 2 * d.W + 2;
  return on && d.KH == 3 && d.KW == 3 && d.stride == 1 && d.pad_t == 1 && d.pad_l == 1 &&
         d.Ho == d.H && d.Wo == d.W && d.Cin % 16 == 0 && !a.rows_in && !a.rows_out &&
         !a.row_count && hp <= 288 && d.H * d.W >= hp &&
         (int64_t)d.N * d.H * d.W * d.Cin_stride < 0x7fffffffLL &&
         (d.prologue == SNAP_PRO_GN_RELU || d.prologue == SNAP_PRO_NONE);
}

template <int BN, int PRO, int NS>
void launch_halo(const ConvArgs& a, dim3 grid, hipStream_t s) {
  const int hp = 128 + 2 * a.d.W + 2;
  if (hp <= 208)
    hipLaunchKernelGGL((conv3x3_halo_kernel<BN, PRO, NS, 208>), grid, dim3(256), 0, s, a);
  else
    hipLaunchKernelGGL((conv3x3_halo_kernel<BN, PRO, NS, 288>), grid, dim3(256), 0, s, a);
}

template <int BM, int BN, int PRO, int NS, bool GNT, bool TAIL, bool DUAL = false, bool PLAIN = false>
__global__ __launch_bounds__(256, NS == 2 ? 4 : 3) void conv_split_kernel(const ConvArgs a) {
  conv_split_body<BM, BN, PRO, NS, GNT, TAIL, false, DUAL, PLAIN>(a);
}

template <int BN, int PRO, int NS>
__global__ __launch_bounds__(256, NS == 2 ? 4 : 3) void conv_split_root_kernel(const ConvArgs a) {
  conv_split_body<128, BN, PRO, NS, false, false, true>(a);
}

template <int BM, int BN, int PRO, int NS>
int launch(ConvArgs a, hipStream_t s) {
  constexpr int BK = 16;
  a.ctiles = (a.d.Cin + BK - 1) / BK;
  a.nk = a.d.KH * a.d.KW * a.ctiles;
  const int64_t nrow = snap_cdiv(a.M, BM);
  a.ncol = (int)snap_cdiv(a.d.Cout, BN);
  a.gn_slabs = (a.d.Ho * a.d.Wo) / BM + 2;
  int64_t nblocks = snap_cdiv(nrow, 8) * 8 * a.ncol;
  if (nblocks > 0x7fffffffLL) return SNAP_ERR_BAD_SHAPE;
  a.ksplit = 1;
  a.tiles_per_split = (int)nblocks;
  a.slabs_per_split = a.nk;
  const int64_t tiles = nrow * a.ncol;
  const int target = splitk_target();
  if (a.kpartial && target > 0 && tiles <= splitk_max_tiles() && a.nk >= 16 && !a.rows_in &&
      !a.rows_out && !a.row_count && (!a.gn_partial || (a.gn_rows32 && a.d.Cout_stride == a.d.Cout)) &&
      !(a.d.epilogue & SNAP_EPI_UPSAMPLE2X_ADD)) {
    int64_t S = (target + tiles - 1) / tiles;
    S = S < a.nk / 8 ? S : a.nk / 8;
    const int64_t fit = (int64_t)(a.kpartial_bytes / ((size_t)a.M * a.d.Cout * sizeof(float)));
    S = S < fit ? S : fit;
    if (S >= 2) {
      a.slabs_per_split = (int)((a.nk + S - 1) / S);
      a.ksplit = (a.nk + a.slabs_per_split - 1) / a.slabs_per_split;
      nblocks *= a.ksplit;
    }
  }
  if (a.gn_partial && a.gn_rows32 && a.ksplit == 1) return SNAP_ERR_WORKSPACE;
  constexpr bool need_gn = (PRO == SNAP_PRO_GN_RELU || PRO == SNAP_PRO_RELU_GN);
  const bool table_ok = !need_gn || (a.d.Ho * a.d.Wo >= BM && !a.rows_in);
  const bool tail = (a.d.Cin & 3) != 0;
  const dim3 grid((unsigned)nblocks);
  if constexpr (BM == 128 && (PRO == SNAP_PRO_GN_RELU || PRO == SNAP_PRO_NONE)) {
    if (halo_ok(a)) {
      if (a.ksplit > 1) {
        const int per = (a.ctiles + a.ksplit - 1) / a.ksplit;
        ConvArgs h = a;
        h.slabs_per_split = per;
        h.ksplit = (a.ctiles + per - 1) / per;
        if (h.ksplit > 1) {
          const dim3 hgrid((unsigned)(h.tiles_per_split * h.ksplit));
          launch_halo<BN, PRO, NS>(h, hgrid, s);
          SNAP_CHECK_LAUNCH();
          return launch_splitk_reduce(h, s);
        }
        if (h.gn_partial) return SNAP_ERR_UNSUPPORTED;
        h.ksplit = 1;
        h.slabs_per_split = h.nk;
        launch_halo<BN, PRO, NS>(h, dim3((unsigned)h.tiles_per_split), s);
        SNAP_CHECK_LAUNCH();
        return SNAP_OK;
      }
      launch_halo<BN, PRO, NS>(a, grid, s);
      SNAP_CHECK_LAUNCH();
      return SNAP_OK;
    }
  }
  bool dual = false;
  if constexpr (BM == 128 && BN == 128 && PRO == SNAP_PRO_GN_RELU)
    dual = a.gn_partial2 != nullptr && a.gn_partial != nullptr && table_ok && a.ksplit == 1;
  if (a.gn_partial2_done) *a.gn_partial2_done = dual ? 1 : 0;
  if constexpr (BM == 128 && BN == 128 && PRO == SNAP_PRO_GN_RELU) {
    if (dual) {
      hipLaunchKernelGGL((conv_split_kernel<BM, BN, PRO, NS, true, false, true>), grid, dim3(256), 0, s, a);
      SNAP_CHECK_LAUNCH();
      return SNAP_OK;
    }
  }
  const bool plain = !a.no_plain && a.d.KH == 1 && a.d.KW == 1 && a.d.stride == 1 && a.d.pad_t == 0 &&
                     a.d.pad_l == 0 && a.d.H == a.d.Ho && a.d.W == a.d.Wo && a.d.Cin % 16 == 0 &&
                     (a.d.Cin_stride & 3) == 0 && !a.rows_in && !a.row_count && a.M > 0 &&
                     (int64_t)BM * a.d.Cin_stride * 4 < 0x7ff00000LL;
  if constexpr (NS == 2 && (PRO == SNAP_PRO_GN_RELU || PRO == SNAP_PRO_NONE || PRO == SNAP_PRO_RELU_GN)) {
    if (plain && (!need_gn || table_ok)) {
      hipLaunchKernelGGL((conv_split_kernel<BM, BN, PRO, NS, need_gn, false, false, true>), grid, dim3(256), 0, s, a);
      SNAP_CHECK_LAUNCH();
      return a.ksplit > 1 ? launch_splitk_reduce(a, s) : SNAP_OK;
    }
  }
  if (need_gn && table_ok)
    hipLaunchKernelGGL((conv_split_kernel<BM, BN, PRO, NS, need_gn, false>), grid, dim3(256), 0, s, a);
  else if (tail)
    hipLaunchKernelGGL((conv_split_kernel<BM, BN, PRO, NS, false, true>), grid, dim3(256), 0, s, a);
  else
    hipLaunchKernelGGL((conv_split_kernel<BM, BN, PRO, NS, false, false>), grid, dim3(256), 0, s, a);
  SNAP_CHECK_LAUNCH();
  return a.ksplit > 1 ? launch_splitk_reduce(a, s) : SNAP_OK;
}

template <int BM, int BN, int NS>
int launch_pro(const ConvArgs& a, hipStream_t s) {
  switch (a.d.prologue) {
    case SNAP_PRO_NONE: return launch<BM, BN, SNAP_PRO_NONE, NS>(a, s);
    case SNAP_PRO_AFFINE: return launch<BM, BN, SNAP_PRO_AFFINE, NS>(a, s);
    case SNAP_PRO_GN_RELU: return launch<BM, BN, SNAP_PRO_GN_RELU, NS>(a, s);
    case SNAP_PRO_RELU_GN: return launch<BM, BN, SNAP_PRO_RELU_GN, NS>(a, s);
    case SNAP_PRO_RELU: return launch<BM, BN, SNAP_PRO_RELU, NS>(a, s);
    default: return SNAP_ERR_UNSUPPORTED;
  }
}

template <int NS>
int launch_tile(const ConvArgs& a, hipStream_t s) {
  const TileChoice t = choose_tile(a.M, a.d.Cout, a.d.tile_hint, desc_k(a.d));
  if (t.bm == 128 && t.bn == 128) return launch_pro<128, 128, NS>(a, s);
  if (t.bm == 128) return launch_pro<128, 64, NS>(a, s);
  if (t.bn == 128) return launch_pro<64, 128, NS>(a, s);
  return launch_pro<64, 64, NS>(a, s);
}

__device__ __forceinline__ void pack_weights_split_body(const float* __restrict__ w,
                                                        __bf16* __restrict__ out, int taps, int Cin,
                                                        int ctiles, int Cout, int parts, int bx,
                                                        int by, int t) {
  __shared__ float tile[32][33];
  const int tx = threadIdx.x & 31, ty = threadIdx.x >> 5;
  const int c0 = bx * 32, n0 = by * 32;
#pragma unroll
  for (int j = ty; j < 32; j += 8) {
    const int c = c0 + j, n = n0 + tx;
    tile[j][tx] = (c < Cin && n < Cout) ? w[((int64_t)t * Cin + c) * Cout + n] : 0.f;
  }
  __syncthreads();
  for (int i = threadIdx.x; i < 128 * parts; i += 256) {
    const int p = i >> 7, q = i & 127;
    const int j = q >> 2, slab = (q >> 1) & 1, ko = q & 1;
    const int n = n0 + j, cb = c0 + 16 * slab;
    if (cb >= 16 * ctiles) continue;
    const int col = n & 127;
    const int oct = ko ^ ((col >> 3) & 1);
    const int64_t blk = ((int64_t)(n >> 7) * taps + t) * ctiles + (cb >> 4);
    bf16x8 v;
#pragma unroll
    for (int e = 0; e < 8; ++e) {
      float r = tile[16 * slab + 8 * ko + e][j];
      for (int pp = 0; pp < p; ++pp) r -= (float)(__bf16)r;
      v[e] = (__bf16)r;
    }
    *reinterpret_cast<bf16x8*>(out + blk * ((int64_t)parts * 2048) + p * 2048 + col * 16 + oct * 8) = v;
  }
}

__global__ __launch_bounds__(256) void pack_weights_split_kernel(
    const float* __restrict__ w, __bf16* __restrict__ out, int taps, int Cin, int ctiles, int Cout,
    int parts) {
  pack_weights_split_body(w, out, taps, Cin, ctiles, Cout, parts, blockIdx.x, blockIdx.y, blockIdx.z);
}

__global__ __launch_bounds__(256) void pack_weights_split_multi_kernel(
    const SnapPackItem* __restrict__ items, int n_items, int parts) {
  int lo = 0, hi = n_items - 1;
  while (lo < hi) {
    const int mid = (lo + hi + 1) >> 1;
    if (items[mid].block_begin <= (int)blockIdx.x) lo = mid; else hi = mid - 1;
  }
  const SnapPackItem it = items[lo];
  const int ctiles = (it.Cin + 15) / 16;
  const int gx = (16 * ctiles + 31) / 32;
  const int gy = ((it.Cout + 127) / 128 * 128) / 32;
  const int local = blockIdx.x - it.block_begin;
  const int t = local / (gx * gy);
  const int rem = local - t * (gx * gy);
  pack_weights_split_body(it.w, static_cast<__bf16*>(it.out), it.taps, it.Cin, ctiles, it.Cout, parts,
                          rem % gx, rem / gx, t);
}

__global__ __launch_bounds__(256) void pack_weights_split_root_kernel(const float* __restrict__ w,
                                                                      __bf16* __restrict__ out,
                                                                      int Cout, int cout128, int parts) {
  const int i = blockIdx.x * 256 + threadIdx.x;
  if (i >= 14 * cout128 * 16) return;
  const int k = i & 15;
  const int n = (i >> 4) % cout128;
  const int t = i / (16 * cout128);
  const int kh = t >> 1, kw = 4 * (t & 1) + (k >> 2), c = k & 3;
  float r = (kw < 7 && c < 3 && n < Cout) ? w[((kh * 7 + kw) * 3 + c) * Cout + n] : 0.f;
  const int col = n & 127;
  const int oct = (k >> 3) ^ ((col >> 3) & 1);
  __bf16* o = out + ((int64_t)(n >> 7) * 14 + t) * ((int64_t)parts * 2048) + col * 16 + oct * 8 + (k & 7);
  for (int p = 0; p < parts; ++p) {
    const __bf16 b = (__bf16)r;
    o[p * 2048] = b;
    r -= (float)b;
  }
}

}

namespace {
template <int BN, int NS>
int launch_root_pro(const ConvArgs& a, dim3 grid, hipStream_t s) {
  if (a.d.prologue == SNAP_PRO_AFFINE)
    hipLaunchKernelGGL((conv_split_root_kernel<BN, SNAP_PRO_AFFINE, NS>), grid, dim3(256), 0, s, a);
  else if (a.d.prologue == SNAP_PRO_NONE)
    hipLaunchKernelGGL((conv_split_root_kernel<BN, SNAP_PRO_NONE, NS>), grid, dim3(256), 0, s, a);
  else
    return SNAP_ERR_UNSUPPORTED;
  SNAP_CHECK_LAUNCH();
  return SNAP_OK;
}
}

int snapconv::launch_split_root(ConvArgs a, int parts, hipStream_t s) {
  const SnapConvDesc& d = a.d;
  if (d.KH != 7 || d.KW != 7 || d.stride != 2 || d.pad_t != 3 || d.pad_l != 3 || d.Cin != 3 ||
      d.Cin_stride != 4 || a.rows_in || a.rows_out || a.row_count || a.gn_partial)
    return SNAP_ERR_UNSUPPORTED;
  if (parts == 2 && d.Cout == 64 && d.Cout_stride == 64 && hint_mode(d.tile_hint) != 1 &&
      (d.prologue == SNAP_PRO_AFFINE || d.prologue == SNAP_PRO_NONE) && !(d.epilogue & ~SNAP_EPI_RELU) &&
      (a.M >= 40000 || hint_mode(d.tile_hint) == 2 || hint_mode(d.tile_hint) == 4) && d.W >= 8)
    return launch_root_ws(a, s);
  a.d.KW = 2;
  a.ctiles = 1;
  a.nk = 14;
  a.ksplit = 1;
  a.slabs_per_split = a.nk;
  const bool wide = d.Cout > 64;
  const int bn = wide ? 128 : 64;
  a.ncol = (int)snap_cdiv(d.Cout, bn);
  a.gn_slabs = (d.Ho * d.Wo) / 128 + 2;
  const int64_t nblocks = snap_cdiv(snap_cdiv(a.M, 128), 8) * 8 * a.ncol;
  if (nblocks > 0x7fffffffLL) return SNAP_ERR_BAD_SHAPE;
  a.tiles_per_split = (int)nblocks;
  const dim3 grid((unsigned)nblocks);
  if (parts == 2) return wide ? launch_root_pro<128, 2>(a, grid, s) : launch_root_pro<64, 2>(a, grid, s);
  if (parts == 3) return wide ? launch_root_pro<128, 3>(a, grid, s) : launch_root_pro<64, 3>(a, grid, s);
  return SNAP_ERR_UNSUPPORTED;
}

int snapconv::launch_split(ConvArgs a, int parts, hipStream_t s) {
  const int kind = stationary_kind(a.d, parts, a.rows_in || a.rows_out || a.row_count);
  if (kind && a.gn_partial && a.gn_rows32) return SNAP_ERR_WORKSPACE;
  switch (kind) {
    case 1: return launch_rs(a, s);
    case 2: case 3: return launch_bs(a, s);
    default: break;
  }
  if (parts == 2) return launch_tile<2>(a, s);
  if (parts == 3) return launch_tile<3>(a, s);
  return SNAP_ERR_UNSUPPORTED;
}

extern "C" size_t snap_conv2d_packed_weights_split_bytes(int32_t taps, int32_t Cin, int32_t Cout,
                                                         int32_t parts) {
  if (parts < 1 || parts > 3 || taps <= 0 || Cin <= 0 || Cout <= 0) return 0;
  const size_t cin16 = ((size_t)Cin + 15) / 16 * 16;
  const size_t cout128 = ((size_t)Cout + 127) / 128 * 128;
  const size_t elems = (size_t)parts * cout128 * taps * cin16;
  if (elems >= ((size_t)1 << 33)) return 0;
  return elems * 2;
}

extern "C" int snap_conv2d_pack_weights_split_bf16(const float* w, int32_t taps, int32_t Cin,
                                                   int32_t Cout, int32_t parts, void* out,
                                                   size_t out_bytes, void* stream) {
  if (!w || !out) return SNAP_ERR_NULL;
  if (taps <= 0 || Cin <= 0 || Cout <= 0) return SNAP_ERR_BAD_SHAPE;
  if (parts < 1 || parts > 3) return SNAP_ERR_UNSUPPORTED;
  const size_t need = snap_conv2d_packed_weights_split_bytes(taps, Cin, Cout, parts);
  if (need == 0) return SNAP_ERR_UNSUPPORTED;
  if (out_bytes < need) return SNAP_ERR_WORKSPACE;
  if (reinterpret_cast<uintptr_t>(out) & 15) return SNAP_ERR_BAD_SHAPE;
  const int ctiles = (Cin + 15) / 16;
  const int cout128 = (Cout + 127) / 128 * 128;
  const dim3 grid((unsigned)snap_cdiv(16 * ctiles, 32), (unsigned)(cout128 / 32), (unsigned)taps);
  hipLaunchKernelGGL(pack_weights_split_kernel, grid, dim3(256), 0, static_cast<hipStream_t>(stream),
                     w, static_cast<__bf16*>(out), taps, Cin, ctiles, Cout, parts);
  SNAP_CHECK_LAUNCH();
  return SNAP_OK;
}

extern "C" int32_t snap_conv2d_pack_weights_split_blocks(int32_t taps, int32_t Cin, int32_t Cout) {
  if (taps <= 0 || Cin <= 0 || Cout <= 0) return 0;
  const int ctiles = (Cin + 15) / 16;
  return ((16 * ctiles + 31) / 32) * (((Cout + 127) / 128 * 128) / 32) * taps;
}

extern "C" int snap_conv2d_pack_weights_split_multi_bf16(const SnapPackItem* items, int32_t n_items,
                                                         int32_t total_blocks, int32_t parts,
                                                         void* stream) {
  if (!items) return SNAP_ERR_NULL;
  if (n_items <= 0 || total_blocks <= 0) return SNAP_ERR_BAD_SHAPE;
  if (parts < 1 || parts > 3) return SNAP_ERR_UNSUPPORTED;
  hipLaunchKernelGGL(pack_weights_split_multi_kernel, dim3((unsigned)total_blocks), dim3(256), 0,
                     static_cast<hipStream_t>(stream), items, n_items, parts);
  SNAP_CHECK_LAUNCH();
  return SNAP_OK;
}

extern "C" size_t snap_conv2d_packed_weights_split_root_bytes(int32_t Cout, int32_t parts) {
  if (parts < 2 || parts > 3 || Cout <= 0) return 0;
  return (size_t)parts * ((Cout + 127) / 128 * 128) * 14 * 16 * 2;
}

extern "C" int snap_conv2d_pack_weights_split_root_bf16(const float* w, int32_t Cout, int32_t parts,
                                                        void* out, size_t out_bytes, void* stream) {
  if (!w || !out) return SNAP_ERR_NULL;
  const size_t need = snap_conv2d_packed_weights_split_root_bytes(Cout, parts);
  if (need == 0) return SNAP_ERR_UNSUPPORTED;
  if (out_bytes < need) return SNAP_ERR_WORKSPACE;
  if (reinterpret_cast<uintptr_t>(out) & 15) return SNAP_ERR_BAD_SHAPE;
  const int cout128 = (Cout + 127) / 128 * 128;
  hipLaunchKernelGGL(pack_weights_split_root_kernel, dim3((unsigned)snap_cdiv(14 * cout128 * 16, 256)),
                     dim3(256), 0, static_cast<hipStream_t>(stream), w, static_cast<__bf16*>(out),
                     Cout, cout128, parts);
  SNAP_CHECK_LAUNCH();
  return SNAP_OK;
}
```

### snap_amd/ops.py

```python
import contextlib
import operator
import sys
import ctypes
import threading
import typing
import weakref
import os

import numpy as np
import torch

from snap_amd import _lib

PRO_NONE, PRO_AFFINE, PRO_GN_RELU, PRO_RELU_GN, PRO_RELU = (
    _lib.SNAP_PRO_NONE, _lib.SNAP_PRO_AFFINE, _lib.SNAP_PRO_GN_RELU, _lib.SNAP_PRO_RELU_GN, _lib.SNAP_PRO_RELU)
EPI_BIAS, EPI_RELU, EPI_RESIDUAL, EPI_UPSAMPLE2X_ADD, EPI_ROWMASK, EPI_GELU = (
    _lib.SNAP_EPI_BIAS, _lib.SNAP_EPI_RELU, _lib.SNAP_EPI_RESIDUAL, _lib.SNAP_EPI_UPSAMPLE2X_ADD,
    _lib.SNAP_EPI_ROWMASK, _lib.SNAP_EPI_GELU)
POOLING = {'max': _lib.SNAP_POOL_MAX, 'sum': _lib.SNAP_POOL_SUM, 'mean': _lib.SNAP_POOL_MEAN}
SIM_CHUNK = _lib.SNAP_SIM_CHUNK



_TUNING_DEFAULTS = {
    'OVERLAP_AERIAL': True,
    'POOLED_SPLIT': True,
    'CLASS_ROWS': True,
    'LIFT_IN_CONSUMER': True,
    'MLP_GATHER_XCD_GROUP': 8,
    'NATIVE_GLUE': True,
    'USE_PRESPLIT': False,
    'CONV_TILE': None,
    'CONV_BK': None,
    'CONV_NO_HALO': False,
    'CONV_NO_RS': False,
    'CONV_RS_NSPLIT': 0,
    'CONV_RS_FORCE': False,
    'CONV_NO_WS': False,
    'SPLITK_STATS': True,
    'CONV_NO_PLAIN': False,
    'USE_PRESPLIT_VOTING': True,
    'PS_RES_INIT': True,
    'PS_TILE': 0,
    'BF16_PS': True,
    'USE_FUSED_GN_STATS': True,
    'GN_STATS_BOTH': True,
    'USE_SPLITK': True,
    'FUSED_TEMPLATE_PACK': True,
    'SIM_GENERAL_KERNEL': False,
    'LATTICE_WINDOW': True,
    'WGRAD_SIDE_STREAM': True,
    'FUSE_STEM': True,
}


class Tuning:
  __slots__ = tuple(_TUNING_DEFAULTS)

  def __init__(self, **kw):
    for k, v in _TUNING_DEFAULTS.items():
      object.__setattr__(self, k, kw.pop(k, v))
    if kw:
      raise TypeError(f'Tuning: unknown switch(es) {sorted(kw)}')

  def replace(self, **kw):
    vals = {k: getattr(self, k) for k in _TUNING_DEFAULTS}
    for k in kw:
      if k not in vals:
        raise TypeError(f'Tuning: unknown switch {k!r}')
    vals.update(kw)
    return Tuning(**vals)

  def __repr__(self):
    diff = {k: getattr(self, k) for k, v in _TUNING_DEFAULTS.items() if getattr(self, k) != v}
    return 'Tuning(' + ', '.join(f'{k}={v!r}' for k, v in diff.items()) + ')'


_DEFAULT_TUNING = Tuning()
_TUNING_TLS = threading.local()


def tuning():
  t = getattr(_TUNING_TLS, 'tuning', None)
  return _DEFAULT_TUNING if t is None else t


@contextlib.contextmanager
def tuning_scope(base=None, **overrides):
  prev = getattr(_TUNING_TLS, 'tuning', None)
  _TUNING_TLS.tuning = (base if base is not None else tuning()).replace(**overrides)
  try:
    yield _TUNING_TLS.tuning
  finally:
    _TUNING_TLS.tuning = prev


_raw_stream = getattr(torch._C, '_cuda_getCurrentRawStream', None)
_raw_device = getattr(torch._C, '_cuda_getDevice', None)


def _stream():
  if _raw_stream is not None and _raw_device is not None:
    return ctypes.c_void_p(_raw_stream(_raw_device()))
  return ctypes.c_void_p(torch.cuda.current_stream().cuda_stream)


_SIDE_STREAMS = {}


def side_stream(device=None):
  idx = torch.cuda.current_device() if device is None else torch.device(device).index
  if idx is None:
    idx = torch.cuda.current_device()
  s = _SIDE_STREAMS.get(idx)
  if s is None:
    s = _SIDE_STREAMS[idx] = torch.cuda.Stream(device=idx)
  return s


class KernelProfiler:

  def __init__(self):
    self.records = {}

  def region(self, name, flops=0.0, nbytes=0.0, tag=None):
    return _Region(self, name, flops, nbytes, tag)

  def launches(self, name):
    torch.cuda.synchronize()
    return [
        (r[4], r[0].elapsed_time(r[1]), _num(r[2]), _num(r[3]))
        for r in self.records.get(name, [])
    ]

  def summary(self):
    torch.cuda.synchronize()
    out = {}
    for name, recs in self.records.items():
      ms = sum(r[0].elapsed_time(r[1]) for r in recs)
      out[name] = dict(
          launches=len(recs), ms=ms, flops=sum(_num(r[2]) for r in recs),
          bytes=sum(_num(r[3]) for r in recs),
      )
    return out


def _num(v):
  return float(v()) if callable(v) else v


class _Region:

  def __init__(self, prof, name, flops, nbytes, tag=None):
    self.prof, self.name, self.flops, self.nbytes, self.tag = prof, name, flops, nbytes, tag

  def __enter__(self):
    self.start = torch.cuda.Event(enable_timing=True)
    self.start.record()

  def __exit__(self, *exc):
    end = torch.cuda.Event(enable_timing=True)
    end.record()
    self.prof.records.setdefault(self.name, []).append(
        (self.start, end, self.flops, self.nbytes, self.tag)
    )


class _NoRegion:

  def __enter__(self):
    pass

  def __exit__(self, *exc):
    pass


_PROFILER = None
_NO_REGION = _NoRegion()


def set_profiler(prof):
  global _PROFILER
  old, _PROFILER = _PROFILER, prof
  return old


def _region(name, flops=0.0, nbytes=0.0, tag=None):
  if _PROFILER is None:
    return _NO_REGION
  return _PROFILER.region(name, flops, nbytes, tag() if callable(tag) else tag)


def _p(t):
  if t is None:
    return None
  return ctypes.c_void_p(t.data_ptr())


def _pv(t):
  return None if t is None else t.data_ptr()


_PIN_RING = []
_PIN_NEXT = 0


_PIN_LOCK = threading.Lock()


def upload_table(items, device):
  raw = np.ascontiguousarray(items).view(np.uint8).reshape(-1)
  device = torch.device(device)
  if device.type != 'cuda':
    return torch.from_numpy(raw.copy()).to(device)
  global _PIN_NEXT
  n = raw.size
  with _PIN_LOCK:
    if not _PIN_RING:
      _PIN_RING.extend([torch.empty(1 << 17, dtype=torch.uint8, pin_memory=True), None] for _ in range(16))
    slot = _PIN_RING[_PIN_NEXT % 16]
    _PIN_NEXT += 1
    if slot[1] is not None:
      slot[1].synchronize()
    if slot[0].numel() < n:
      slot[0] = torch.empty(n, dtype=torch.uint8, pin_memory=True)
    slot[0][:n].numpy()[:] = raw
    out = slot[0][:n].to(device, non_blocking=True)
    ev = torch.cuda.Event()
    ev.record()
    slot[1] = ev
  return out


_HOST_SCALARS = {}


def prefetch_exp(t):
  if t is None or not t.is_cuda:
    return
  prev = _HOST_SCALARS.get(id(t))
  if prev is not None and prev[0]() is t:
    host = prev[2]
    prev[3].synchronize()
  else:
    host = torch.empty(1, dtype=torch.float32, pin_memory=True)
  host.copy_(torch.exp(t.detach().to(torch.float32)).reshape(1), non_blocking=True)
  ev = torch.cuda.Event()
  ev.record()
  if len(_HOST_SCALARS) > 64:
    _HOST_SCALARS.clear()
  _HOST_SCALARS[id(t)] = (weakref.ref(t), t._version, host, ev)


def host_exp(t):
  hit = _HOST_SCALARS.get(id(t))
  if hit is not None and hit[0]() is t and hit[1] == t._version:
    hit[3].synchronize()
    return float(hit[2][0])
  return float(torch.exp(t.detach().to(torch.float32)))


def _chk(t, dtype, name):
  if not isinstance(t, torch.Tensor):
    raise TypeError(f'{name}: expected a torch.Tensor, got {type(t)}')
  if not t.is_cuda:
    raise RuntimeError(
        f'{name}: tensor is on {t.device}; snap_amd ops run only on a ROCm GPU '
        '(no CPU fallback).'
    )
  if t.dtype != dtype:
    raise TypeError(f'{name}: expected {dtype}, got {t.dtype}')
  if not t.is_contiguous():
    raise ValueError(f'{name}: tensor must be contiguous')
  return t


def _f32(t, name):
  return _chk(t, torch.float32, name)


def _mask(t, name):
  if t.dtype == torch.bool:
    return _chk(t, torch.bool, name)
  return _chk(t, torch.uint8, name)


def _arg_chk(t, name, dtypes, shape, device, want, also=True, tail=''):
  if (not isinstance(t, torch.Tensor) or t.dtype not in dtypes
      or (not t.is_cuda if device is None else t.device != device) or t.dim() != len(shape)
      or any(s is not None and s != d for s, d in zip(shape, t.shape)) or not also):
    got = f'{t.dtype} {tuple(t.shape)} on {t.device}' if isinstance(t, torch.Tensor) else type(t)
    raise ValueError(f'{want}, got {got}{tail}')
  return _chk(t, t.dtype, name)


def _workspace_words(nbytes_fn, args, numel, unsupported):
  nbytes = nbytes_fn(*args) if numel < 2 ** 31 else 0
  if nbytes == 0:
    raise ValueError(unsupported)
  return nbytes // 8


class PreSplit:

  def __init__(self, data, shape):
    self.data = data
    self.shape = tuple(shape)
    self.device = data.device

  def numel(self):
    return int(np.prod(self.shape))


def gn_norm_split(y, gamma, beta, *, groups=32, eps=1e-5, want_stats=False):
  fused = getattr(y, '_snap_gn_partial', None)
  N, H, W, C = y.shape
  if (precision() != 'bf16x3' or fused is None or fused[2] or groups != 32
      or C % 16 or C > 2048 or not tuning().USE_FUSED_GN_STATS):
    return None
  lib = _lib.load()
  _f32(y, 'y'); _f32(gamma, 'gamma'); _f32(beta, 'beta')
  partial, tile_rows, _ = fused
  out = torch.empty(y.numel() * 2, dtype=torch.bfloat16, device=y.device)
  mu = sc = None
  if want_stats:
    mu = torch.empty((N, C), dtype=torch.float32, device=y.device)
    sc = torch.empty((N, C), dtype=torch.float32, device=y.device)
  with _region('gn_norm_split', 0.0, 8.0 * y.numel()):
    st = lib.snap_gn_norm_split_f32(_p(y), _p(partial), N, H * W, C, groups, eps, tile_rows,
                                    _p(gamma), _p(beta), _p(out), _p(mu), _p(sc), _stream())
  _lib.check(st, 'snap_gn_norm_split_f32')
  ps = PreSplit(out, (N, H, W, C))
  if want_stats:
    ps.stats = (mu, sc)
  return ps


def presplit(x):
  lib = _lib.load()
  _f32(x, 'x')
  C = x.shape[-1]
  rows = x.numel() // C
  out = torch.empty(x.numel() * 2, dtype=torch.bfloat16, device=x.device)
  with _region('presplit', 0.0, 8.0 * x.numel()):
    st = lib.snap_presplit_f32(_p(x), rows, C, _p(out), _stream())
  _lib.check(st, 'snap_presplit_f32')
  shape = tuple(x.shape) if x.dim() == 4 else (1,) * (4 - x.dim()) + tuple(x.shape)
  return PreSplit(out, shape)


def _stationary_mode(T=None):
  T = tuning() if T is None else T
  if T.CONV_NO_RS:
    return 1
  if T.CONV_RS_FORCE:
    return 4 if T.CONV_NO_WS else 2
  return 3 if T.CONV_NO_WS else 0


class PackedWeights:

  def __init__(self, data, shape):
    self.data = data
    self.shape = tuple(int(v) for v in shape)

  def numel(self):
    return int(np.prod(self.shape))


def pack_stacked_templates_split(templates, S):
  lib = _lib.load()
  _f32(templates, 'templates')
  R, H, W, D = templates.shape
  KH, KW, RS = H + S - 1, W + S - 1, R * S * S
  nbytes = lib.snap_conv2d_packed_weights_split_bytes(KH * KW, D, RS, 2)
  if nbytes == 0:
    return None
  out = torch.empty(nbytes // 2, dtype=torch.bfloat16, device=templates.device)
  with _region('pack_stacked_templates', 0.0, 4.0 * templates.numel() + float(nbytes)):
    st = lib.snap_pack_stacked_templates_split_bf16(_p(templates), H, W, D, R, S, _p(out), nbytes, _stream())
  _lib.check(st, 'snap_pack_stacked_templates_split_bf16')
  return PackedWeights(out, (KH, KW, D, RS))


HALF_MATH = ('bf16', 'fp16')
SPLIT_PARTS = {'bf16x3': 2, 'bf16x6': 3}


def kernel_image(w_shape, math):
  KH, KW, Cin, Cout = w_shape
  parts = SPLIT_PARTS.get(math, 0)
  if parts and _lib.load().snap_conv2d_packed_weights_split_bytes(KH * KW, Cin, Cout, parts) == 0:
    math, parts = 'f32', 0
  return math, parts, math != 'f32' and Cin >= 4


def conv2d_presplit_supported(x_shape, w_shape, stride=1, padding=((0, 0), (0, 0))):
  lib = _lib.load()
  N, H, W, Cs = x_shape
  KH, KW, Cin, Cout = w_shape
  (pt, pb), (pl, pr) = padding
  if Cs != Cin or Cin % 16:
    return False
  Ho = (H + pt + pb - KH) // stride + 1
  Wo = (W + pl + pr - KW) // stride + 1
  if Ho <= 0 or Wo <= 0:
    return False
  if kernel_image(w_shape, 'bf16x3')[1] != 2:
    return False
  d = _lib.SnapConvDesc(N, H, W, Cin, Cs, KH, KW, stride, pt, pl, Ho, Wo, Cout, Cout, PRO_NONE, 0, 1.0, 0.0)
  return bool(lib.snap_conv2d_presplit_supported(ctypes.byref(d)))


class ConvPlan(typing.NamedTuple):
  desc: _lib.SnapConvDesc
  out_shape: tuple
  out_dtype: torch.dtype
  engine: str
  family: str
  tag: str
  image: str
  parts: int
  extras: bool
  workspace_bytes: int
  stats_bytes: int
  stats_count: int
  stats_relu: bool
  gn_partial_rows: int
  tile_rows: int
  gnb: bool
  w_split_parts: int
  w_split_root: int
  w_half: int
  x_half: int
  x_presplit: int
  ps_tile: int
  ps_res_init: int
  bk_hint: int
  tune_flags: int


def plan_conv(
    x, w, stride=1, padding=((0, 0), (0, 0)), cin=None, prologue=PRO_NONE,
    gn=None, in_affine=(1.0, 0.0), bias=None, relu=False, residual=None,
    up_prev=None, row_mask=None, rows_in=None, rows_out=None, row_count=None, out=None,
    emit_gn_stats=None, math=None, gelu=False, res_init=None, ps_tile=None, out_half=False, out_stride=None,
    gn_bwd_stats=None, bf16_ring=False,
):
  lib = _lib.load()
  T = tuning()
  ps = isinstance(x, PreSplit)
  pw = isinstance(w, PackedWeights)
  xh = (not ps) and x.dtype in (torch.bfloat16, torch.float16)
  no_rows = rows_in is None and rows_out is None and row_count is None
  if xh:
    want = 'fp16' if x.dtype == torch.float16 else 'bf16'
    math = want if math is None else math
    if (math != want or prologue != PRO_NONE or rows_in is not None or x.shape[-1] % 8 or w.shape[2] % 8
        or emit_gn_stats is not None):
      raise ValueError('conv2d: a half-precision input takes the matching engine, prologue NONE, whole '
                       'channel octets, no input row list / statistics')
  if ps:
    if prologue != PRO_NONE or not no_rows or math not in (None, 'bf16x3'):
      raise ValueError('conv2d: a PreSplit input takes prologue NONE, no row lists, math bf16x3')
    math = 'bf16x3'
  if pw and not ps:
    raise ValueError('conv2d: PackedWeights (a two-part split image) go with a PreSplit input')
  N, H, W, Cs = x.shape
  KH, KW, Cin, Cout = w.shape
  if cin is None:
    cin = Cs
  if cin != Cin:
    raise ValueError(f'conv2d: kernel expects Cin={Cin}, input has {cin}')
  (pt, pb), (pl, pr) = padding
  Ho = (H + pt + pb - KH) // stride + 1
  Wo = (W + pl + pr - KW) // stride + 1
  M = N * Ho * Wo
  out_dtype = torch.float32
  if out_half:
    hm = precision() if math is None else math
    if (hm not in HALF_MATH or out is not None or emit_gn_stats is not None or up_prev is not None
        or prologue not in (PRO_NONE, PRO_RELU) or Cs % 4 or Cin < 4 or Cout % 4):
      raise ValueError('conv2d: out_half needs a training-precision engine launch (prologue NONE / RELU, '
                       'no statistics / up-sampling epilogue, channel quads)')
    out_dtype = torch.float16 if hm == 'fp16' else torch.bfloat16
  elif out is not None:
    if out_stride is not None:
      if (out_stride % 4 or out_stride < Cout or out.numel() != M * out_stride or emit_gn_stats is not None
          or residual is not None or up_prev is not None):
        raise ValueError('conv2d: out_stride needs out [rows, out_stride], out_stride % 4 == 0, a plain epilogue')
    elif out.numel() != M * Cout:
      raise ValueError('conv2d: out has the wrong size')
  if out_stride is not None and out is None:
    raise ValueError('conv2d: out_stride goes with out')
  epi = 0
  if prologue in (PRO_GN_RELU, PRO_RELU_GN):
    mu, sc, beta = gn
    if mu.numel() != N * Cin or sc.numel() != N * Cin or beta.numel() != Cin:
      raise ValueError('conv2d: GroupNorm statistics have the wrong size')
  if bias is not None:
    epi |= EPI_BIAS
    if bias.numel() != Cout:
      raise ValueError('conv2d: bias size')
  if relu:
    epi |= EPI_RELU
  if gelu:
    epi |= EPI_GELU
  if residual is not None:
    epi |= EPI_RESIDUAL
    y_shape = (N, Ho, Wo, Cout) if out is None else tuple(out.shape)
    if tuple(residual.shape) != y_shape:
      raise ValueError(f'conv2d: residual {tuple(residual.shape)} vs {y_shape}')
  if up_prev is not None:
    epi |= EPI_UPSAMPLE2X_ADD
    if tuple(up_prev.shape) != (N, Ho // 2, Wo // 2, Cout):
      raise ValueError('conv2d: up_prev shape')
  if row_mask is not None:
    epi |= EPI_ROWMASK
    if row_mask.numel() != M:
      raise ValueError('conv2d: row_mask size')
  tile_hint = 1000000 * _stationary_mode(T)
  if T.CONV_TILE:
    bm, bn = (int(v) for v in T.CONV_TILE.split('x'))
    tile_hint += bm * 1000 + bn
  d = _lib.SnapConvDesc(
      N, H, W, Cin, Cs, KH, KW, stride, pt, pl, Ho, Wo, Cout, Cout if out_stride is None else int(out_stride), prologue,
      epi, float(in_affine[0]), float(in_affine[1]), tile_hint,
  )
  dref = ctypes.byref(d)
  math = precision() if math is None else math
  if math not in ENGINES:
    raise ValueError(f'conv2d: math={math!r}')
  math, parts, packed = kernel_image((KH, KW, Cin, Cout), math)
  packed = packed and Cs % 4 == 0
  qparts = parts if packed and not ps else 0
  ps1 = bool(bf16_ring and xh and x.dtype == torch.bfloat16 and math == 'bf16' and T.BF16_PS and Cs == Cin and Cin % 16 == 0
             and rows_out is None and row_count is None and up_prev is None and gn_bwd_stats is None
             and out is None and Cout % 4 == 0 and lib.snap_conv2d_presplit_supported(dref))
  if xh and out_half and not ps1:
    raise ValueError('conv2d: a half-precision input AND output need the one-part pre-split engine (bf16, Cin % 16 == 0, '
                     'no row lists)')
  kind = lib.snap_conv2d_stationary_kind(dref, qparts) if (qparts == 2 and no_rows) else 0
  pst = (T.PS_TILE if ps_tile is None else int(ps_tile)) if (ps or ps1) else 0
  wbytes = sbytes = scount = rows32 = tile_rows = 0
  gnb = False
  if no_rows:
    if ps:
      wbytes = lib.snap_conv2d_presplit_workspace_bytes(dref, pst) if T.USE_SPLITK else 0
    elif not (ps1 or kind or out_half):
      wbytes = lib.snap_conv2d_workspace_bytes(dref) if T.USE_SPLITK else 0
    if wbytes:
      half_engine = math in HALF_MATH and packed and Cin % 4 == 0 and not ps
      if emit_gn_stats is not None and (qparts >= 2 or half_engine) and T.SPLITK_STATS:
        sbytes = lib.snap_conv2d_splitk_gn_partial_bytes(dref)
        if sbytes:
          scount, rows32, tile_rows = 1, 32, 32
    elif (gn_bwd_stats is not None and xh and emit_gn_stats is None and out is None and up_prev is None
          and not relu and not gelu and row_mask is None):
      gx, gmu, grs, gga, gbe, gmode = gn_bwd_stats
      pbytes = lib.snap_conv2d_gn_partial_bytes_ex(dref, 0)
      if (pbytes and tuple(gx.shape) == (N, Ho, Wo, Cout) and gmu.numel() == N * Cout and grs.numel() == N * Cout
          and gga.numel() == Cout and gbe.numel() == Cout and gmode in (PRO_GN_RELU, PRO_RELU_GN)):
        sbytes, scount, gnb = pbytes, 1, True
        tile_rows = lib.snap_conv2d_tile_rows_ex(dref, 0)
    elif emit_gn_stats is not None:
      sbytes = (lib.snap_conv2d_presplit_gn_partial_bytes(dref, pst) if ps
                else lib.snap_conv2d_gn_partial_bytes_ex(dref, qparts))
      if sbytes:
        scount = 2 if (emit_gn_stats == 'both' and math in SPLIT_PARTS) else 1
        tile_rows = lib.snap_conv2d_presplit_tile_rows(dref, pst) if ps else lib.snap_conv2d_tile_rows_ex(dref, qparts)
  if ps and (parts != 2 or Cin % 16):
    raise ValueError('conv2d: the pre-split engine needs Cin % 16 == 0 and a two-part weight image')
  family, image, iparts = 'conv_igemm', None, 0
  root = xpre = res0 = 0
  if (parts and (KH, KW, stride, Cin, Cs) == (7, 7, 2, 3, 4) and (pt, pl) == (3, 3)
      and prologue in (PRO_NONE, PRO_AFFINE) and no_rows and not sbytes and not ps):
    family, image, iparts, root = f'conv_split_{math}', math + '/root', parts, 1
  elif ps1:
    family, image, iparts, xpre = 'conv_bf16', 'bf16/ps1', 1, 1
  elif packed:
    family = f'conv_split_{math}' if parts else ('conv_fp16' if math == 'fp16' else 'conv_bf16')
    image, iparts = math, parts
    if ps:
      xpre, res0 = 1, int(T.PS_RES_INIT if res_init is None else bool(res_init))
  bk_hint = tune_flags = 0
  tuned = bool(T.CONV_BK or T.CONV_NO_HALO or T.CONV_RS_NSPLIT or T.CONV_NO_PLAIN)
  if tuned:
    bk_hint = int(T.CONV_BK or 0)
    tune_flags = (_lib.SNAP_TUNE_NO_HALO * int(bool(T.CONV_NO_HALO)) | _lib.SNAP_TUNE_NO_PLAIN * int(bool(T.CONV_NO_PLAIN))
                  | ((int(T.CONV_RS_NSPLIT) & 15) << _lib.SNAP_TUNE_RS_NSPLIT_SHIFT))
  return ConvPlan(
      desc=d, out_shape=(N, Ho, Wo, Cout), out_dtype=out_dtype, engine=math if image else 'f32', family=family,
      tag='PS_' if ps else 'PS1_' if ps1 else ('', 'RS_', 'WS_', 'WS_')[kind], image=image, parts=iparts,
      extras=bool(not no_rows or wbytes or sbytes or image or tuned), workspace_bytes=wbytes,
      stats_bytes=sbytes, stats_count=scount, stats_relu=bool(sbytes) and emit_gn_stats == 'relu',
      gn_partial_rows=rows32, tile_rows=tile_rows, gnb=gnb,
      w_split_parts=iparts, w_split_root=root, w_half=int(image == 'fp16'), x_half=int(xh and not ps1),
      x_presplit=xpre, ps_tile=pst if xpre else 0, ps_res_init=res0, bk_hint=bk_hint, tune_flags=tune_flags)


def conv2d(
    x, w, *, stride=1, padding=((0, 0), (0, 0)), cin=None, prologue=PRO_NONE,
    gn=None, in_affine=(1.0, 0.0), bias=None, relu=False, residual=None,
    up_prev=None, row_mask=None, rows_in=None, rows_out=None, row_count=None, out=None,
    emit_gn_stats=None, math=None, gelu=False, res_init=None, ps_tile=None, out_half=False, out_stride=None,
    gn_bwd_stats=None, bf16_ring=False,
):
  lib = _lib.load()
  ps = isinstance(x, PreSplit)
  pw = isinstance(w, PackedWeights)
  if ps:
    xd = _chk(x.data, torch.bfloat16, 'x')
  else:
    xd = _chk(x, x.dtype if x.dtype in (torch.bfloat16, torch.float16) else torch.float32, 'x')
  wd = w.data if pw else _f32(w, 'w')
  if out is not None:
    _f32(out, 'out')
  for t, nm in ((rows_in, 'rows_in'), (rows_out, 'rows_out'), (row_count, 'row_count')):
    if t is not None:
      _chk(t, torch.int32, nm)
  mu = sc = beta = None
  if prologue in (PRO_GN_RELU, PRO_RELU_GN):
    mu, sc, beta = gn
    _f32(mu, 'gn_mu'); _f32(sc, 'gn_sc'); _f32(beta, 'gn_beta')
  if bias is not None:
    _f32(bias, 'bias')
  if residual is not None:
    _f32(residual, 'residual')
  if up_prev is not None:
    _f32(up_prev, 'up_prev')
  if row_mask is not None:
    _mask(row_mask, 'row_mask')
  p = plan_conv(x, w, stride, padding, cin, prologue, gn, in_affine, bias, relu, residual, up_prev, row_mask, rows_in,
                rows_out, row_count, out, emit_gn_stats, math, gelu, res_init, ps_tile, out_half, out_stride,
                gn_bwd_stats, bf16_ring)
  dev = xd.device
  y = out if out is not None else torch.empty(p.out_shape, dtype=p.out_dtype, device=dev)
  kws = torch.empty(p.workspace_bytes // 4, dtype=torch.float32, device=dev) if p.workspace_bytes else None
  partial = torch.empty(p.stats_bytes // 4, dtype=torch.float32, device=dev) if p.stats_count else None
  partial2 = torch.empty(p.stats_bytes // 4, dtype=torch.float32, device=dev) if p.stats_count == 2 else None
  wpk = None
  if p.image is not None:
    wpk = wd if pw else _packed_weights(w, p.image, p.parts)
  ex = None
  if p.extras:
    ex = _lib.SnapConvExtras()
    if rows_in is not None or rows_out is not None or row_count is not None:
      ex.rows_in, ex.rows_out, ex.row_count = _pv(rows_in), _pv(rows_out), _pv(row_count)
    if kws is not None:
      ex.workspace, ex.workspace_bytes = kws.data_ptr(), p.workspace_bytes
    if partial is not None:
      ex.gn_partial, ex.gn_partial_bytes = partial.data_ptr(), p.stats_bytes
      ex.gn_partial_relu, ex.gn_partial_rows = int(p.stats_relu), p.gn_partial_rows
    if partial2 is not None:
      ex.gn_partial2, ex.gn_partial2_bytes = partial2.data_ptr(), p.stats_bytes
    if p.gnb:
      for t, nm in zip(gn_bwd_stats[:5], ('gn_bwd x', 'gn_bwd mu', 'gn_bwd rstd', 'gn_bwd gamma', 'gn_bwd beta')):
        _f32(t, nm)
      ex.gnb_x, ex.gnb_mu, ex.gnb_rstd, ex.gnb_gamma, ex.gnb_beta = (t.data_ptr() for t in gn_bwd_stats[:5])
      ex.gnb_mode = int(gn_bwd_stats[5])
    if wpk is not None:
      ex.w_bf16, ex.w_bf16_bytes = wpk.data_ptr(), wpk.numel() * 2
      ex.w_split_parts, ex.w_split_root, ex.w_half, ex.x_half = p.w_split_parts, p.w_split_root, p.w_half, p.x_half
      ex.x_presplit, ex.ps_tile, ex.ps_res_init = p.x_presplit, p.ps_tile, p.ps_res_init
      if out_half:
        ex.y_half = y.data_ptr()
    ex.bk_hint, ex.tune_flags = p.bk_hint, p.tune_flags
  N, Ho, Wo, Cout = p.out_shape
  KH, KW, Cin = w.shape[:3]
  M = N * Ho * Wo
  kflops = 2.0 * KH * KW * Cin * Cout
  if row_count is None:
    flops = kflops * M
    nbytes = 4.0 * ((x.numel() if ps else x.numel() * (0.5 if p.x_half or p.image == 'bf16/ps1' else 1.0)) + w.numel() + y.numel()
                    + (residual.numel() if residual is not None else 0))
  else:
    flops = lambda: kflops * int(row_count.item())
    nbytes = lambda: 4.0 * (int(row_count.item()) * (Cin + Cout) + wd.numel())
  with _region(
      p.family, flops, nbytes,
      lambda: f'{p.tag}M{M}{"r" if row_count is not None else ""}_K{KH}x{KW}x{Cin}_N{Cout}_s{stride}_p{prologue}_e{p.desc.epilogue}',
  ):
    st = lib.snap_conv2d_nhwc_ex_f32(
        ctypes.byref(p.desc), _p(xd), _p(wd), None if out_half else _p(y), _p(mu), _p(sc), _p(beta), _p(bias),
        _p(residual), _p(up_prev), _p(row_mask), None if ex is None else ctypes.byref(ex),
        _stream(),
    )
  _lib.check(st, 'snap_conv2d_nhwc_ex_f32')
  if p.gnb:
    y._snap_gnb_partial = (partial, p.tile_rows, gn_bwd_stats[0].data_ptr(), gn_bwd_stats[0]._version, int(gn_bwd_stats[5]))
  elif partial is not None:
    y._snap_gn_partial = (partial, p.tile_rows, p.stats_relu)
    if partial2 is not None and ex.gn_partial2_done:
      y._snap_gn_partial_relu = (partial2, p.tile_rows, True)
  return y


def _root_pool_plan(x, w, cin, prologue, in_affine, relu, math):
  if not tuning().FUSE_STEM or isinstance(x, PreSplit) or isinstance(w, PackedWeights):
    return None
  p = plan_conv(x, w, 2, ((3, 3), (3, 3)), cin, prologue, None, in_affine, None, relu, math=math)
  ok = p.w_split_root and _lib.load().snap_conv2d_root_pool_supported(ctypes.byref(p.desc), p.parts)
  return p if ok else None


def conv2d_root_pool_supported(x, w, *, cin=None, prologue=PRO_NONE, in_affine=(1.0, 0.0), relu=False, math=None):
  return _root_pool_plan(x, w, cin, prologue, in_affine, relu, math) is not None


def conv2d_root_pool(x, w, *, cin=None, prologue=PRO_NONE, in_affine=(1.0, 0.0), relu=False, math=None, band_rows=0):
  p = _root_pool_plan(x, w, cin, prologue, in_affine, relu, math)
  if p is None:
    return max_pool_3x3s2(conv2d(x, w, stride=2, padding=((3, 3), (3, 3)), cin=cin, prologue=prologue,
                                 in_affine=in_affine, relu=relu, math=math))
  lib = _lib.load()
  xd = _f32(x, 'x')
  _f32(w, 'w')
  wpk = _packed_weights(w, p.image, p.parts)
  N, Ho, Wo, Cout = p.out_shape
  y = torch.empty((N, (Ho - 1) // 2 + 1, (Wo - 1) // 2 + 1, Cout), dtype=torch.float32, device=xd.device)
  with _region(p.family, 2.0 * 147 * Cout * N * Ho * Wo, 4.0 * (x.numel() + w.numel() + y.numel()),
               lambda: f'POOL_M{N * Ho * Wo}_K7x7x3_N{Cout}_s2_p{prologue}_e{p.desc.epilogue}'):
    st = lib.snap_conv2d_root_pool_f32(ctypes.byref(p.desc), _p(xd), _p(wpk), wpk.numel() * 2, p.parts, int(band_rows),
                                       _p(y), _stream())
  _lib.check(st, 'snap_conv2d_root_pool_f32')
  return y


def pack_weights_bf16(w, half=False):
  lib = _lib.load()
  _f32(w, 'w')
  KH, KW, Cin, Cout = w.shape
  nbytes = lib.snap_conv2d_packed_weights_bytes(KH * KW, Cin, Cout)
  out = torch.empty(nbytes // 2, dtype=torch.float16 if half else torch.bfloat16, device=w.device)
  fn = lib.snap_conv2d_pack_weights_f16 if half else lib.snap_conv2d_pack_weights_bf16
  st = fn(_p(w), KH * KW, Cin, Cout, _p(out), nbytes, _stream())
  _lib.check(st, 'snap_conv2d_pack_weights_f16' if half else 'snap_conv2d_pack_weights_bf16')
  return out


PACK_EPOCH = 0


def _image_get(w, key, explicit=False):
  slot = getattr(w, '_snap_packed', None)
  hit = None if slot is None else slot.get(key)
  if isinstance(hit, tuple):
    return hit[2] if hit[0] == PACK_EPOCH and hit[1] == w._version else None
  return hit if explicit else None


def _image_put(w, key, image):
  slot = getattr(w, '_snap_packed', None)
  if slot is None:
    slot = w._snap_packed = {}
  slot[key] = (PACK_EPOCH, w._version, image)


def _packed_weights(w, math, parts):
  wpk = _image_get(w, math, explicit=True)
  if wpk is None:
    if math.endswith('/root'):
      wpk = pack_weights_split_root_bf16(w, parts)
    else:
      wpk = pack_weights_split_bf16(w, parts) if parts else pack_weights_bf16(w, half=(math == 'fp16'))
    try:
      _image_put(w, math, wpk)
    except AttributeError:
      pass
  return wpk


def pack_weights_split_bf16(w, parts):
  lib = _lib.load()
  _f32(w, 'w')
  KH, KW, Cin, Cout = w.shape
  nbytes = lib.snap_conv2d_packed_weights_split_bytes(KH * KW, Cin, Cout, parts)
  out = torch.empty(nbytes // 2, dtype=torch.bfloat16, device=w.device)
  st = lib.snap_conv2d_pack_weights_split_bf16(_p(w), KH * KW, Cin, Cout, parts, _p(out), nbytes,
                                               _stream())
  _lib.check(st, 'snap_conv2d_pack_weights_split_bf16')
  return out


def pack_weights_split_root_bf16(w, parts):
  lib = _lib.load()
  _f32(w, 'w')
  if tuple(w.shape[:3]) != (7, 7, 3):
    raise ValueError('pack_weights_split_root_bf16: w must be [7, 7, 3, Cout]')
  Cout = w.shape[3]
  nbytes = lib.snap_conv2d_packed_weights_split_root_bytes(Cout, parts)
  out = torch.empty(nbytes // 2, dtype=torch.bfloat16, device=w.device)
  st = lib.snap_conv2d_pack_weights_split_root_bf16(_p(w), Cout, parts, _p(out), nbytes, _stream())
  _lib.check(st, 'snap_conv2d_pack_weights_split_root_bf16')
  return out


_PACK_ITEM = np.dtype(_lib.SnapPackItem)


def pack_weights_split_multi(ws, math):
  parts = SPLIT_PARTS[math]
  lib = _lib.load()
  todo = [w for w in ws if _image_get(w, math) is None and kernel_image(w.shape, math)[2]]
  if not todo:
    return
  items = np.zeros(len(todo), dtype=_PACK_ITEM)
  outs = []
  blk = 0
  for i, w in enumerate(todo):
    _f32(w, 'w')
    KH, KW, Cin, Cout = w.shape
    nbytes = lib.snap_conv2d_packed_weights_split_bytes(KH * KW, Cin, Cout, parts)
    out = torch.empty(nbytes // 2, dtype=torch.bfloat16, device=w.device)
    outs.append(out)
    items[i] = (w.data_ptr(), out.data_ptr(), KH * KW, Cin, Cout, blk)
    blk += lib.snap_conv2d_pack_weights_split_blocks(KH * KW, Cin, Cout)
  table = upload_table(items, todo[0].device)
  st = lib.snap_conv2d_pack_weights_split_multi_bf16(_p(table), len(todo), blk, parts, _stream())
  _lib.check(st, 'snap_conv2d_pack_weights_split_multi_bf16')
  for w, out in zip(todo, outs):
    _image_put(w, math, out)


def pack_weights_bf16_multi(ws, with_rotated=True, math='bf16'):
  lib = _lib.load()
  if math not in HALF_MATH:
    raise ValueError(f'pack_weights_bf16_multi: math={math!r}')
  half = math == 'fp16'
  todo = [w for w in ws if _image_get(w, math) is None and kernel_image(w.shape, math)[2]]
  if not todo:
    return
  n = len(todo) * (2 if with_rotated else 1)
  items = np.zeros(n, dtype=_PACK_ITEM)
  outs = []
  blk = 0
  i = 0
  for w in todo:
    _f32(w, 'w')
    KH, KW, Cin, Cout = w.shape
    taps = KH * KW
    for rot in ((False, True) if with_rotated else (False,)):
      nbytes = (lib.snap_conv2d_packed_weights_bytes(taps, Cout, (Cin + 3) // 4 * 4) if rot
                else lib.snap_conv2d_packed_weights_bytes(taps, Cin, Cout))
      out = torch.empty(nbytes // 2, dtype=torch.float16 if half else torch.bfloat16, device=w.device)
      outs.append(out)
      items[i] = (w.data_ptr(), out.data_ptr(), -taps if rot else taps, Cin, Cout, blk)
      blk += lib.snap_conv2d_pack_weights_blocks(-taps if rot else taps, Cin, Cout)
      i += 1
  table = upload_table(items, todo[0].device)
  fn = lib.snap_conv2d_pack_weights_multi_f16 if half else lib.snap_conv2d_pack_weights_multi_bf16
  st = fn(_p(table), n, blk, _stream())
  _lib.check(st, 'snap_conv2d_pack_weights_multi_f16' if half else 'snap_conv2d_pack_weights_multi_bf16')
  k = 0
  for w in todo:
    _image_put(w, math, outs[k]); k += 1
    if with_rotated:
      _image_put(w, math + '/rot', outs[k]); k += 1


def packed_rot_image(w, math='bf16'):
  return _image_get(w, math + '/rot')


def dense(x, kernel, bias=None, *, cin=None, prologue=PRO_NONE, relu=False,
          row_mask=None, rows_in=None, rows_out=None, row_count=None, out=None, math=None,
          gelu=False, residual=None, out_half=False, out_stride=None, bf16_ring=False):
  lead = x.shape[:-1]
  M = int(np.prod(lead)) if len(lead) else 1
  strided = out_stride is not None
  y = conv2d(
      x.reshape(1, 1, M, x.shape[-1]), kernel.reshape(1, 1, *kernel.shape),
      cin=cin if cin is not None else kernel.shape[0], prologue=prologue,
      bias=bias, relu=relu, row_mask=row_mask, rows_in=rows_in, rows_out=rows_out,
      row_count=row_count, out=out if (strided or out is None) else out.reshape(1, 1, M, kernel.shape[1]),
      math=math, gelu=gelu, out_stride=out_stride,
      residual=None if residual is None else residual.reshape(1, 1, M, kernel.shape[1]),
      out_half=out_half, bf16_ring=bf16_ring,
  )
  return out if strided else y.reshape(*lead, kernel.shape[1])


def semantic_embed(rasters, idx_road, idx_other, table_road, table_other):
  lib = _lib.load()
  _mask(rasters, 'rasters'); _f32(table_road, 'table_road'); _f32(table_other, 'table_other')
  N = rasters.shape[-1]
  M = rasters.numel() // N
  E = table_road.shape[1]
  nr, no = len(idx_road), len(idx_other)
  if tuple(table_road.shape) != (nr, E) or tuple(table_other.shape) != (2 * no, E):
    raise ValueError('semantic_embed: table shapes')
  ir = (ctypes.c_int32 * max(nr, 1))(*idx_road)
  io = (ctypes.c_int32 * max(no, 1))(*idx_other)
  out = torch.empty((*rasters.shape[:-1], (1 + no) * E), dtype=torch.float32, device=rasters.device)
  st = lib.snap_semantic_embed_f32(_p(rasters), M, N, ctypes.cast(ir, ctypes.c_void_p), nr,
                                   ctypes.cast(io, ctypes.c_void_p), no, _p(table_road),
                                   _p(table_other), E, _p(out), _stream())
  _lib.check(st, 'snap_semantic_embed_f32')
  return out


def semantic_onehot(rasters, idx_road, idx_other):
  lib = _lib.load()
  _mask(rasters, 'rasters')
  N = rasters.shape[-1]
  M = rasters.numel() // N
  nr, no = len(idx_road), len(idx_other)
  KP = (nr + 2 * no + 3) // 4 * 4
  ir = (ctypes.c_int32 * max(nr, 1))(*idx_road)
  io = (ctypes.c_int32 * max(no, 1))(*idx_other)
  onehot = torch.empty((M, KP), dtype=torch.float32, device=rasters.device)
  st = lib.snap_semantic_onehot_f32(_p(rasters), M, N, ctypes.cast(ir, ctypes.c_void_p), nr,
                                    ctypes.cast(io, ctypes.c_void_p), no, _p(onehot), KP, _stream())
  _lib.check(st, 'snap_semantic_onehot_f32')
  return onehot


def stack_templates(tw, S, layout='hwdr'):
  lib = _lib.load()
  _f32(tw, 'tw')
  if layout == 'hwdr':
    H, W, D, R = tw.shape
    fn, name = lib.snap_stack_templates_f32, 'snap_stack_templates_f32'
  else:
    R, H, W, D = tw.shape
    fn, name = lib.snap_stack_templates_rhwd_f32, 'snap_stack_templates_rhwd_f32'
  tws = torch.empty((H + S - 1, W + S - 1, D, R * S * S), dtype=torch.float32, device=tw.device)
  st = fn(_p(tw), _p(tws), H, W, D, R, S, _stream())
  _lib.check(st, name)
  return tws


def layer_norm(x, gamma, beta, eps=1e-6, out_half=False):
  lib = _lib.load()
  _f32(x, 'x'); _f32(gamma, 'gamma'); _f32(beta, 'beta')
  C = x.shape[-1]
  M = x.numel() // C
  if out_half:
    y = torch.empty(x.shape, dtype=torch.bfloat16, device=x.device)
    with _region('layer_norm', 0.0, 6.0 * x.numel()):
      st = lib.snap_layer_norm_bf16out_f32(_p(x), _p(gamma), _p(beta), _p(y), M, C, float(eps), _stream())
    _lib.check(st, 'snap_layer_norm_bf16out_f32')
    return y
  y = torch.empty_like(x)
  with _region('layer_norm', 0.0, 8.0 * x.numel()):
    st = lib.snap_layer_norm_f32(_p(x), _p(gamma), _p(beta), _p(y), M, C, float(eps), _stream())
  _lib.check(st, 'snap_layer_norm_f32')
  return y


def attention(qkv, scale=None, want_lse=False, out_half=False):
  lib = _lib.load()
  B, N, three, H, D = qkv.shape
  if three != 3:
    raise ValueError('attention: qkv must be [B, N, 3, H, D]')
  scale = D ** -0.5 if scale is None else float(scale)
  if qkv.dtype == torch.bfloat16:
    if want_lse or not out_half:
      raise ValueError('attention: a bf16 qkv is the inference form (out_half=True, no lse)')
    _chk(qkv, torch.bfloat16, 'qkv')
    out = torch.empty((B, N, H * D), dtype=torch.bfloat16, device=qkv.device)
    with _region('attention', 4.0 * B * H * N * N * D, 2.0 * (qkv.numel() + out.numel())):
      st = lib.snap_attention_bf16io(_p(qkv), _p(out), B, N, H, D, scale, _stream())
    _lib.check(st, 'snap_attention_bf16io')
    return out
  _f32(qkv, 'qkv')
  if out_half:
    if want_lse:
      raise ValueError('attention: out_half is the inference form (no lse)')
    out = torch.empty((B, N, H * D), dtype=torch.bfloat16, device=qkv.device)
# ... 1544 lines not shown
```

Before: 407.4 scenes/s.

## Close split-K reduction in the last-arriving conv block via atomic tile counters

Replaces the separate split-K reduce kernel launch with an in-kernel close. Each output tile keeps an atomic arrival counter in a persistent per-stream arena, and the last split to arrive sums the partials, applies the epilogue, emits GroupNorm partial stats and resets the counter. This is meant to save a kernel launch and the serialization gap per split-K conv. In exchange, the closing block does the whole reduction serially, and correctness now depends on threadfence ordering and the counters being zeroed. The diff also adds a knob to force a split-K factor.

```diff
diff --git a/include/snap_hip.h b/include/snap_hip.h
--- a/include/snap_hip.h
+++ b/include/snap_hip.h
@@ -79,6 +79,9 @@
 #define SNAP_TUNE_NO_HALO 1
 #define SNAP_TUNE_NO_PLAIN 8
 #define SNAP_TUNE_RS_NSPLIT_SHIFT 4
+#define SNAP_TUNE_SPLITK_CLOSE 256
+#define SNAP_SPLITK_COUNTER_BYTES 2048
+#define SNAP_TUNE_SPLITK_SHIFT 12
 int32_t snap_conv2d_presplit_tile_rows(const SnapConvDesc* desc, int32_t ps_tile);
 size_t snap_conv2d_presplit_gn_partial_bytes(const SnapConvDesc* desc, int32_t ps_tile);
 size_t snap_conv2d_presplit_workspace_bytes(const SnapConvDesc* desc, int32_t ps_tile);
diff --git a/snap_amd/csrc/conv_common.h b/snap_amd/csrc/conv_common.h
--- a/snap_amd/csrc/conv_common.h
+++ b/snap_amd/csrc/conv_common.h
@@ -24,7 +24,10 @@
   const int32_t* row_count;
   float* kpartial;
   size_t kpartial_bytes;
+  int* kcount;
   int ksplit;
+  int kclose;
+  int ksplit_force;
   int slabs_per_split;
   int tiles_per_split;
   float* gn_partial;
@@ -83,7 +86,222 @@
   return x / (1.0f + __expf(-2.0f * u));
 }
 
-template <int BM, int BN, bool DUAL = false, int NT = 256, bool SKIP_RES = false, int OUTH = 0, bool GNB = false>
+
+template <int RB>
+__device__ __forceinline__ void splitk_sum_rows(const float* partial, int S, int64_t M, int Cout,
+                                                const int64_t (&m)[RB], int col, f32x4 (&v)[RB]) {
+#pragma unroll
+  for (int k = 0; k < RB; ++k) v[k] = *reinterpret_cast<const f32x4*>(partial + m[k] * Cout + col);
+  int s = 1;
+  if constexpr (RB == 1) {
+    for (; s + 3 < S; s += 4) {
+      f32x4 t[4];
+#pragma unroll
+      for (int u = 0; u < 4; ++u)
+        t[u] = *reinterpret_cast<const f32x4*>(partial + ((int64_t)(s + u) * M + m[0]) * Cout + col);
+#pragma unroll
+      for (int u = 0; u < 4; ++u)
+#pragma unroll
+        for (int e = 0; e < 4; ++e) v[0][e] += t[u][e];
+    }
+  }
+  for (; s < S; ++s) {
+    f32x4 t[RB];
+#pragma unroll
+    for (int k = 0; k < RB; ++k)
+      t[k] = *reinterpret_cast<const f32x4*>(partial + ((int64_t)s * M + m[k]) * Cout + col);
+#pragma unroll
+    for (int k = 0; k < RB; ++k)
+#pragma unroll
+      for (int e = 0; e < 4; ++e) v[k][e] += t[k][e];
+  }
+}
+
+__device__ __forceinline__ f32x4 splitk_finish(f32x4 v, int epi, const f32x4& bb, const f32x4& rr, bool masked) {
+  if (epi & SNAP_EPI_BIAS) {
+#pragma unroll
+    for (int e = 0; e < 4; ++e) v[e] += bb[e];
+  }
+  if (epi & SNAP_EPI_RESIDUAL) {
+#pragma unroll
+    for (int e = 0; e < 4; ++e) v[e] += rr[e];
+  }
+  if (epi & SNAP_EPI_RELU) {
+#pragma unroll
+    for (int e = 0; e < 4; ++e) v[e] = snap_relu(v[e]);
+  }
+  if (epi & SNAP_EPI_GELU) {
+#pragma unroll
+    for (int e = 0; e < 4; ++e) v[e] = snap_gelu_tanh(v[e]);
+  }
+  if (masked) v = f32x4{0.f, 0.f, 0.f, 0.f};
+  return v;
+}
+
+struct SplitkClose {
+  const float* partial;
+  int S;
+  int64_t M;
+  int Cout, Cout_stride, epi;
+  const float* bias;
+  const float* residual;
+  const uint8_t* row_mask;
+  float* y;
+  int HoWo, N, gn_slabs, gn_relu;
+  float* gn_partial;
+};
+
+template <int RB>
+__device__ __forceinline__ void splitk_close_slab(const SplitkClose& c, int64_t m0, int64_t m_split, int col,
+                                                  int tp, int PW, float (&s1)[2][4], float (&s2)[2][4]) {
+  for (int r0 = tp; r0 < 32; r0 += RB * PW) {
+    f32x4 v[RB];
+    bool ok[RB];
+    int64_t mr[RB];
+#pragma unroll
+    for (int k = 0; k < RB; ++k) {
+      const int64_t m = m0 + r0 + k * PW;
+      ok[k] = r0 + k * PW < 32 && m < c.M;
+      mr[k] = ok[k] ? m : m0;
+    }
+    splitk_sum_rows<RB>(c.partial, c.S, c.M, c.Cout, mr, col, v);
+    f32x4 bb = {0.f, 0.f, 0.f, 0.f};
+    if (c.epi & SNAP_EPI_BIAS) bb = *reinterpret_cast<const f32x4*>(c.bias + col);
+    f32x4 rr[RB];
+#pragma unroll
+    for (int k = 0; k < RB; ++k) rr[k] = bb;
+    if (c.epi & SNAP_EPI_RESIDUAL) {
+#pragma unroll
+      for (int k = 0; k < RB; ++k)
+        rr[k] = *reinterpret_cast<const f32x4*>(c.residual + mr[k] * c.Cout_stride + col);
+    }
+#pragma unroll
+    for (int k = 0; k < RB; ++k) {
+      if (!ok[k]) continue;
+      const int64_t m = mr[k];
+      v[k] = splitk_finish(v[k], c.epi, bb, rr[k], (c.epi & SNAP_EPI_ROWMASK) && c.row_mask[m] == 0);
+      *reinterpret_cast<f32x4*>(c.y + m * c.Cout_stride + col) = v[k];
+      const int sl = m >= m_split ? 1 : 0;
+#pragma unroll
+      for (int e = 0; e < 4; ++e) {
+        const float t = c.gn_relu ? snap_relu(v[k][e]) : v[k][e];
+        s1[sl][e] += t;
+        s2[sl][e] += t * t;
+      }
+    }
+  }
+}
+
+__device__ __forceinline__ void splitk_stats_park(float* red, int slot, const float (&s1)[2][4], const float (&s2)[2][4]) {
+#pragma unroll
+  for (int sl = 0; sl < 2; ++sl)
+#pragma unroll
+    for (int e = 0; e < 4; ++e) {
+      red[slot * 16 + sl * 8 + e] = s1[sl][e];
+      red[slot * 16 + sl * 8 + 4 + e] = s2[sl][e];
+    }
+}
+
+__device__ __forceinline__ void splitk_stats_store(const SplitkClose& c, const float* red, int slot0, int stride, int PW,
+                                                   int64_t m0, int n_first, int64_t m_split, int col) {
+#pragma unroll
+  for (int sl = 0; sl < 2; ++sl) {
+    const int n = n_first + sl;
+    const bool live = n < c.N && (sl == 0 || (m0 + 32 > m_split && m_split < c.M));
+    if (!live) continue;
+    const int slab = (int)((m0 >> 5) - (((int64_t)n * c.HoWo) >> 5));
+    float* o = c.gn_partial + (((int64_t)n * c.gn_slabs + slab) * c.Cout + col) * 2;
+#pragma unroll
+    for (int e = 0; e < 4; ++e) {
+      float t1 = 0.f, t2 = 0.f;
+      for (int pp = 0; pp < PW; ++pp) {
+        t1 += red[(slot0 + pp * stride) * 16 + sl * 8 + e];
+        t2 += red[(slot0 + pp * stride) * 16 + sl * 8 + 4 + e];
+      }
+      o[2 * e] = t1;
+      o[2 * e + 1] = t2;
+    }
+  }
+}
+
+__global__ __launch_bounds__(256) void splitk_reduce_kernel(
+    const float* __restrict__ partial, int S, int64_t M, int Cout, int Cout_stride, int epi,
+    const float* __restrict__ bias, const float* __restrict__ residual,
+    const uint8_t* __restrict__ row_mask, float* __restrict__ y) {
+  const int Q = Cout >> 2;
+  const int64_t i = (int64_t)blockIdx.x * blockDim.x + threadIdx.x;
+  if (i >= M * Q) return;
+  const int64_t m[1] = {i / Q};
+  const int col = 4 * (int)(i - m[0] * Q);
+  f32x4 v[1];
+  splitk_sum_rows<1>(partial, S, M, Cout, m, col, v);
+  const int64_t o = m[0] * Cout_stride + col;
+  f32x4 bb = {0.f, 0.f, 0.f, 0.f}, rr = bb;
+  if (epi & SNAP_EPI_BIAS) bb = *reinterpret_cast<const f32x4*>(bias + col);
+  if (epi & SNAP_EPI_RESIDUAL) rr = *reinterpret_cast<const f32x4*>(residual + o);
+  *reinterpret_cast<f32x4*>(y + o) = splitk_finish(v[0], epi, bb, rr, (epi & SNAP_EPI_ROWMASK) && row_mask[m[0]] == 0);
+}
+
+__global__ __launch_bounds__(256) void splitk_reduce_stats_kernel(
+    const float* __restrict__ partial, int S, int64_t M, int Cout, int epi,
+    const float* __restrict__ bias, const float* __restrict__ residual,
+    const uint8_t* __restrict__ row_mask, float* __restrict__ y, int HoWo, int N, int gn_slabs,
+    int gn_relu, float* __restrict__ gn_partial) {
+  __shared__ float red[256 * 16];
+  const SplitkClose c = {partial, S, M, Cout, Cout, epi, bias, residual, row_mask, y, HoWo, N, gn_slabs, gn_relu, gn_partial};
+  const int Q = Cout >> 2;
+  const int QW = Q < 256 ? Q : 256;
+  const int PW = 256 / QW;
+  const int tq = threadIdx.x % QW, tp = threadIdx.x / QW;
+  const int64_t m0 = (int64_t)blockIdx.x * 32;
+  const int n_first = (int)(m0 / HoWo);
+  const int64_t m_split = (int64_t)(n_first + 1) * HoWo;
+  for (int q0 = 0; q0 < Q; q0 += QW) {
+    const int q = q0 + tq;
+    const int col = 4 * q;
+    float s1[2][4] = {{0.f, 0.f, 0.f, 0.f}, {0.f, 0.f, 0.f, 0.f}};
+    float s2[2][4] = {{0.f, 0.f, 0.f, 0.f}, {0.f, 0.f, 0.f, 0.f}};
+    if (q < Q && tp < PW) splitk_close_slab<8>(c, m0, m_split, col, tp, PW, s1, s2);
+    __syncthreads();
+    splitk_stats_park(red, threadIdx.x, s1, s2);
+    __syncthreads();
+    if (tp == 0 && q < Q) splitk_stats_store(c, red, tq, QW, PW, m0, n_first, m_split, col);
+  }
+}
+
+template <int BM, int BN>
+__device__ __noinline__ void splitk_close_tile(const SplitkClose& c, float* red, int m0, int n0) {
+  constexpr int QT = BN / 4;
+  const int tid = threadIdx.x;
+  const bool stats = c.gn_partial != nullptr;
+  const int Q = c.Cout >> 2;
+  const int QW = Q < 256 ? Q : 256;
+  const int QTe = stats ? (QT < QW ? QT : QW) : QT;
+  const int PW = stats ? 256 / QW : 256 / QT;
+  const int per = QTe * PW;
+  const int SC = 256 / per;
+  const int tq = tid % QTe, tp = (tid / QTe) % PW, ss = tid / per;
+  const int col = n0 + 4 * tq;
+  for (int sb0 = 0; sb0 < BM / 32; sb0 += SC) {
+    const int sb = sb0 + ss;
+    const int64_t ms = (int64_t)m0 + 32 * sb;
+    const bool act = sb < BM / 32 && ms < c.M && col < c.Cout;
+    const int n_first = (int)(ms / c.HoWo);
+    const int64_t m_split = (int64_t)(n_first + 1) * c.HoWo;
+    float s1[2][4] = {{0.f, 0.f, 0.f, 0.f}, {0.f, 0.f, 0.f, 0.f}};
+    float s2[2][4] = {{0.f, 0.f, 0.f, 0.f}, {0.f, 0.f, 0.f, 0.f}};
+    if (act) splitk_close_slab<4>(c, ms, m_split, col, tp, PW, s1, s2);
+    if (stats) {
+      __syncthreads();
+      splitk_stats_park(red, tid, s1, s2);
+      __syncthreads();
+      if (act && tp == 0) splitk_stats_store(c, red, ss * per + tq, QTe, PW, ms, n_first, m_split, col);
+    }
+  }
+}
+
+template <int BM, int BN, bool DUAL = false, int NT = 256, bool SKIP_RES = false, int OUTH = 0, bool GNB = false,
+          bool CLOSE = false>
 __device__ __forceinline__ void conv_epilogue(const ConvArgs& a,
                                               f32x16 (&acc)[BM / (NT / 4)][BN / 64],
                                               float* smem, int m0, int n0, int Meff, int row_t,
@@ -234,6 +452,24 @@
       }
     }
   }
+  if constexpr (CLOSE) {
+    static_assert(NT == 256, "the closing epilogue is laid out for 256 threads");
+    if (a.ksplit > 1 && a.kcount) {
+      __shared__ int arrived;
+      __threadfence();
+      __syncthreads();
+      int* const cnt = a.kcount + row_t * a.ncol + n0 / BN;
+      if (tid == 0) arrived = atomicAdd(cnt, 1);
+      __syncthreads();
+      if (arrived != a.ksplit - 1) return;
+      __threadfence();
+      const SplitkClose c = {a.kpartial, a.ksplit, (int64_t)a.M, d.Cout, d.Cout_stride, epi, a.bias, a.residual,
+                             a.row_mask, a.y, HoWo, d.N, HoWo / 32 + 2, a.gn_relu, a.gn_partial};
+      splitk_close_tile<BM, BN>(c, smem, m0, n0);
+      if (tid == 0) atomicExch(cnt, 0);
+      return;
+    }
+  }
   if (want_stats) {
     constexpr int RG = NT / Q;
     const int q = tid % Q, rg = tid / Q;
@@ -269,168 +505,8 @@
   }
 }
 
-__global__ __launch_bounds__(256) void splitk_reduce_kernel(
-    const float* __restrict__ partial, int S, int64_t M, int Cout, int Cout_stride, int epi,
-    const float* __restrict__ bias, const float* __restrict__ residual,
-    const uint8_t* __restrict__ row_mask, float* __restrict__ y) {
-  const int Q = Cout >> 2;
-  const int64_t i = (int64_t)blockIdx.x * blockDim.x + threadIdx.x;
-  if (i >= M * Q) return;
-  const int64_t m = i / Q;
-  const int col = 4 * (int)(i - m * Q);
-  f32x4 v = *reinterpret_cast<const f32x4*>(partial + m * Cout + col);
-  int s = 1;
-  for (; s + 3 < S; s += 4) {
-    f32x4 t[4];
-#pragma unroll
-    for (int u = 0; u < 4; ++u)
-      t[u] = *reinterpret_cast<const f32x4*>(partial + ((int64_t)(s + u) * M + m) * Cout + col);
-#pragma unroll
-    for (int u = 0; u < 4; ++u)
-#pragma unroll
-      for (int e = 0; e < 4; ++e) v[e] += t[u][e];
-  }
-  for (; s < S; ++s) {
-    const f32x4 t = *reinterpret_cast<const f32x4*>(partial + ((int64_t)s * M + m) * Cout + col);
-#pragma unroll
-    for (int e = 0; e < 4; ++e) v[e] += t[e];
-  }
-  const int64_t o = m * Cout_stride + col;
-  if (epi & SNAP_EPI_BIAS) {
-    const f32x4 bb = *reinterpret_cast<const f32x4*>(bias + col);
-#pragma unroll
-    for (int e = 0; e < 4; ++e) v[e] += bb[e];
-  }
-  if (epi & SNAP_EPI_RESIDUAL) {
-    const f32x4 rr = *reinterpret_cast<const f32x4*>(residual + o);
-#pragma unroll
-    for (int e = 0; e < 4; ++e) v[e] += rr[e];
-  }
-  if (epi & SNAP_EPI_RELU) {
-#pragma unroll
-    for (int e = 0; e < 4; ++e) v[e] = snap_relu(v[e]);
-  }
-  if (epi & SNAP_EPI_GELU) {
-#pragma unroll
-    for (int e = 0; e < 4; ++e) v[e] = snap_gelu_tanh(v[e]);
-  }
-  if ((epi & SNAP_EPI_ROWMASK) && row_mask[m] == 0) v = f32x4{0.f, 0.f, 0.f, 0.f};
-  *reinterpret_cast<f32x4*>(y + o) = v;
-}
-
-__global__ __launch_bounds__(256) void splitk_reduce_stats_kernel(
-    const float* __restrict__ partial, int S, int64_t M, int Cout, int epi,
-    const float* __restrict__ bias, const float* __restrict__ residual,
-    const uint8_t* __restrict__ row_mask, float* __restrict__ y, int HoWo, int N, int gn_slabs,
-    int gn_relu, float* __restrict__ gn_partial) {
-  __shared__ float red[256 * 16];
-  const int Q = Cout >> 2;
-  const int QW = Q < 256 ? Q : 256;
-  const int PW = 256 / QW;
-  const int tq = threadIdx.x % QW, tp = threadIdx.x / QW;
-  const int64_t m0 = (int64_t)blockIdx.x * 32;
-  const int n_first = (int)(m0 / HoWo);
-  const int64_t m_split = (int64_t)(n_first + 1) * HoWo;
-  for (int q0 = 0; q0 < Q; q0 += QW) {
-    const int q = q0 + tq;
-    const int col = 4 * q;
-    float s1[2][4] = {{0.f, 0.f, 0.f, 0.f}, {0.f, 0.f, 0.f, 0.f}};
-    float s2[2][4] = {{0.f, 0.f, 0.f, 0.f}, {0.f, 0.f, 0.f, 0.f}};
-    if (q < Q && tp < PW) {
-      constexpr int RB = 8;
-      for (int r0 = tp; r0 < 32; r0 += RB * PW) {
-        f32x4 v[RB];
-        bool ok[RB];
-#pragma unroll
-        for (int k = 0; k < RB; ++k) {
-          const int64_t m = m0 + r0 + k * PW;
-          ok[k] = r0 + k * PW < 32 && m < M;
-          v[k] = *reinterpret_cast<const f32x4*>(partial + (ok[k] ? m : m0) * Cout + col);
-        }
-        for (int sp = 1; sp < S; ++sp) {
-          f32x4 t[RB];
-#pragma unroll
-          for (int k = 0; k < RB; ++k)
-            t[k] = *reinterpret_cast<const f32x4*>(partial + ((int64_t)sp * M + (ok[k] ? m0 + r0 + k * PW : m0)) * Cout + col);
-#pragma unroll
-          for (int k = 0; k < RB; ++k)
-#pragma unroll
-            for (int e = 0; e < 4; ++e) v[k][e] += t[k][e];
-        }
-        f32x4 bb = {0.f, 0.f, 0.f, 0.f};
-        if (epi & SNAP_EPI_BIAS) bb = *reinterpret_cast<const f32x4*>(bias + col);
-        f32x4 rr[RB];
-        if (epi & SNAP_EPI_RESIDUAL) {
-#pragma unroll
-          for (int k = 0; k < RB; ++k)
-            rr[k] = *reinterpret_cast<const f32x4*>(residual + (ok[k] ? m0 + r0 + k * PW : m0) * Cout + col);
-        }
-#pragma unroll
-        for (int k = 0; k < RB; ++k) {
-          if (!ok[k]) continue;
-          const int64_t m = m0 + r0 + k * PW;
-          const int64_t o = m * Cout + col;
-          if (epi & SNAP_EPI_BIAS) {
-#pragma unroll
-            for (int e = 0; e < 4; ++e) v[k][e] += bb[e];
-          }
-          if (epi & SNAP_EPI_RESIDUAL) {
-#pragma unroll
-            for (int e = 0; e < 4; ++e) v[k][e] += rr[k][e];
-          }
-          if (epi & SNAP_EPI_RELU) {
-#pragma unroll
-            for (int e = 0; e < 4; ++e) v[k][e] = snap_relu(v[k][e]);
-          }
-          if (epi & SNAP_EPI_GELU) {
-#pragma unroll
-            for (int e = 0; e < 4; ++e) v[k][e] = snap_gelu_tanh(v[k][e]);
-          }
-          if ((epi & SNAP_EPI_ROWMASK) && row_mask[m] == 0) v[k] = f32x4{0.f, 0.f, 0.f, 0.f};
-          *reinterpret_cast<f32x4*>(y + o) = v[k];
-          const int sl = m >= m_split ? 1 : 0;
-#pragma unroll
-          for (int e = 0; e < 4; ++e) {
-            const float t = gn_relu ? snap_relu(v[k][e]) : v[k][e];
-            s1[sl][e] += t;
-            s2[sl][e] += t * t;
-          }
-        }
-      }
-    }
-    __syncthreads();
-#pragma unroll
-    for (int sl = 0; sl < 2; ++sl)
-#pragma unroll
-      for (int e = 0; e < 4; ++e) {
-        red[threadIdx.x * 16 + sl * 8 + e] = s1[sl][e];
-        red[threadIdx.x * 16 + sl * 8 + 4 + e] = s2[sl][e];
-      }
-    __syncthreads();
-    if (tp == 0 && q < Q) {
-#pragma unroll
-      for (int sl = 0; sl < 2; ++sl) {
-        const int n = n_first + sl;
-        const bool live = n < N && (sl == 0 || (m0 + 32 > m_split && m_split < M));
-        if (!live) continue;
-        const int slab = (int)(blockIdx.x - (((int64_t)n * HoWo) >> 5));
-        float* o = gn_partial + (((int64_t)n * gn_slabs + slab) * Cout + col) * 2;
-#pragma unroll
-        for (int e = 0; e < 4; ++e) {
-          float t1 = 0.f, t2 = 0.f;
-          for (int pp = 0; pp < PW; ++pp) {
-            t1 += red[(pp * QW + tq) * 16 + sl * 8 + e];
-            t2 += red[(pp * QW + tq) * 16 + sl * 8 + 4 + e];
-          }
-          o[2 * e] = t1;
-          o[2 * e + 1] = t2;
-        }
-      }
-    }
-  }
-}
-
 inline int launch_splitk_reduce(const ConvArgs& a, hipStream_t s) {
+  if (a.kcount) return SNAP_OK;
   if (a.gn_partial) {
     if (!a.gn_rows32 || (a.d.Cout & 3) || (256 % ((a.d.Cout >> 2) < 256 ? (a.d.Cout >> 2) : 256)) != 0)
       return SNAP_ERR_UNSUPPORTED;
@@ -450,6 +526,7 @@
 
 constexpr int64_t splitk_max_tiles() { return 384; }
 constexpr int splitk_target() { return 768; }
+constexpr int splitk_counter_ints() { return SNAP_SPLITK_COUNTER_BYTES / 4; }
 
 struct TileChoice { int bm, bn; };
 inline int hint_tile(int h) { return h % 1000000; }
diff --git a/snap_amd/csrc/conv_igemm.hip b/snap_amd/csrc/conv_igemm.hip
--- a/snap_amd/csrc/conv_igemm.hip
+++ b/snap_amd/csrc/conv_igemm.hip
@@ -630,6 +630,9 @@
   a.kpartial_bytes = ex ? ex->workspace_bytes : 0;
   if (reinterpret_cast<uintptr_t>(a.kpartial) & 15) a.kpartial = nullptr;
   a.ksplit = 1; a.slabs_per_split = 0; a.tiles_per_split = 0;
+  a.kcount = nullptr;
+  a.kclose = (ex && (ex->tune_flags & SNAP_TUNE_SPLITK_CLOSE)) ? 1 : 0;
+  a.ksplit_force = ex ? (ex->tune_flags >> SNAP_TUNE_SPLITK_SHIFT) & 15 : 0;
   a.gn_slabs = 0;
   a.M = d.N * d.Ho * d.Wo;
   a.K = d.KH * d.KW * d.Cin;
diff --git a/snap_amd/csrc/conv_split.hip b/snap_amd/csrc/conv_split.hip
--- a/snap_amd/csrc/conv_split.hip
+++ b/snap_amd/csrc/conv_split.hip
@@ -3,7 +3,8 @@
 namespace {
 
 
-template <int BM, int BN, int PRO, int NS, bool GNT, bool TAIL, bool ROOT = false, bool DUAL = false, bool PLAIN = false>
+template <int BM, int BN, int PRO, int NS, bool GNT, bool TAIL, bool ROOT = false, bool DUAL = false, bool PLAIN = false,
+          bool CLOSE = false>
 __device__ __forceinline__ void conv_split_body(const ConvArgs& a) {
   constexpr int BK = 16;
   constexpr int TM = BM / 64;
@@ -267,10 +268,10 @@
     __syncthreads();
   }
 
-  conv_epilogue<BM, BN, DUAL>(a, acc, smem, m0, n0, Meff, row_t, split);
-}
-
-template <int BN, int PRO, int NS, int HPMAX>
+  conv_epilogue<BM, BN, DUAL, 256, false, 0, false, CLOSE>(a, acc, smem, m0, n0, Meff, row_t, split);
+}
+
+template <int BN, int PRO, int NS, int HPMAX, bool CLOSE = false>
 __device__ __forceinline__ void conv3x3_halo_body(const ConvArgs& a) {
   constexpr int BM = 128, BK = 16;
   constexpr int TM = 2, TN = BN / 64;
@@ -479,12 +480,12 @@
       bcur ^= 1;
     }
   }
-  conv_epilogue<BM, BN>(a, acc, smem, m0, n0, Meff, row_t, split);
-}
-
-template <int BN, int PRO, int NS, int HPMAX>
+  conv_epilogue<BM, BN, false, 256, false, 0, false, CLOSE>(a, acc, smem, m0, n0, Meff, row_t, split);
+}
+
+template <int BN, int PRO, int NS, int HPMAX, bool CLOSE = false>
 __global__ __launch_bounds__(256, NS == 2 ? 3 : 2) void conv3x3_halo_kernel(const ConvArgs a) {
-  conv3x3_halo_body<BN, PRO, NS, HPMAX>(a);
+  conv3x3_halo_body<BN, PRO, NS, HPMAX, CLOSE>(a);
 }
 
 inline bool halo_ok(const ConvArgs& a) {
@@ -501,15 +502,19 @@
 template <int BN, int PRO, int NS>
 void launch_halo(const ConvArgs& a, dim3 grid, hipStream_t s) {
   const int hp = 128 + 2 * a.d.W + 2;
-  if (hp <= 208)
-    hipLaunchKernelGGL((conv3x3_halo_kernel<BN, PRO, NS, 208>), grid, dim3(256), 0, s, a);
-  else
-    hipLaunchKernelGGL((conv3x3_halo_kernel<BN, PRO, NS, 288>), grid, dim3(256), 0, s, a);
-}
-
-template <int BM, int BN, int PRO, int NS, bool GNT, bool TAIL, bool DUAL = false, bool PLAIN = false>
+  const bool close = a.ksplit > 1 && a.kcount;
+  if (hp <= 208) {
+    if (close) hipLaunchKernelGGL((conv3x3_halo_kernel<BN, PRO, NS, 208, true>), grid, dim3(256), 0, s, a);
+    else hipLaunchKernelGGL((conv3x3_halo_kernel<BN, PRO, NS, 208>), grid, dim3(256), 0, s, a);
+  } else {
+    if (close) hipLaunchKernelGGL((conv3x3_halo_kernel<BN, PRO, NS, 288, true>), grid, dim3(256), 0, s, a);
+    else hipLaunchKernelGGL((conv3x3_halo_kernel<BN, PRO, NS, 288>), grid, dim3(256), 0, s, a);
+  }
+}
+
+template <int BM, int BN, int PRO, int NS, bool GNT, bool TAIL, bool DUAL = false, bool PLAIN = false, bool CLOSE = false>
 __global__ __launch_bounds__(256, NS == 2 ? 4 : 3) void conv_split_kernel(const ConvArgs a) {
-  conv_split_body<BM, BN, PRO, NS, GNT, TAIL, false, DUAL, PLAIN>(a);
+  conv_split_body<BM, BN, PRO, NS, GNT, TAIL, false, DUAL, PLAIN, CLOSE>(a);
 }
 
 template <int BN, int PRO, int NS>
@@ -532,11 +537,20 @@
   a.slabs_per_split = a.nk;
   const int64_t tiles = nrow * a.ncol;
   const int target = splitk_target();
-  if (a.kpartial && target > 0 && tiles <= splitk_max_tiles() && a.nk >= 16 && !a.rows_in &&
+  a.kcount = nullptr;
+  if (a.kclose && a.kpartial && tiles <= splitk_counter_ints() &&
+      a.kpartial_bytes > (size_t)SNAP_SPLITK_COUNTER_BYTES) {
+    a.kcount = reinterpret_cast<int*>(a.kpartial);
+    a.kpartial += splitk_counter_ints();
+    a.kpartial_bytes -= SNAP_SPLITK_COUNTER_BYTES;
+  }
+  const bool forced = a.ksplit_force > 1;
+  if (a.kpartial && target > 0 && (forced || (tiles <= splitk_max_tiles() && a.nk >= 16)) && !a.rows_in &&
       !a.rows_out && !a.row_count && (!a.gn_partial || (a.gn_rows32 && a.d.Cout_stride == a.d.Cout)) &&
       !(a.d.epilogue & SNAP_EPI_UPSAMPLE2X_ADD)) {
     int64_t S = (target + tiles - 1) / tiles;
     S = S < a.nk / 8 ? S : a.nk / 8;
+    if (forced) S = a.ksplit_force < a.nk ? a.ksplit_force : a.nk;
     const int64_t fit = (int64_t)(a.kpartial_bytes / ((size_t)a.M * a.d.Cout * sizeof(float)));
     S = S < fit ? S : fit;
     if (S >= 2) {
@@ -545,6 +559,8 @@
       nblocks *= a.ksplit;
     }
   }
+  if (a.ksplit == 1 || (a.d.Cin & 3) != 0) a.kcount = nullptr;
+  const bool close = a.kcount != nullptr;
   if (a.gn_partial && a.gn_rows32 && a.ksplit == 1) return SNAP_ERR_WORKSPACE;
   constexpr bool need_gn = (PRO == SNAP_PRO_GN_RELU || PRO == SNAP_PRO_RELU_GN);
   const bool table_ok = !need_gn || (a.d.Ho * a.d.Wo >= BM && !a.rows_in);
@@ -592,12 +608,20 @@
                      (int64_t)BM * a.d.Cin_stride * 4 < 0x7ff00000LL;
   if constexpr (NS == 2 && (PRO == SNAP_PRO_GN_RELU || PRO == SNAP_PRO_NONE || PRO == SNAP_PRO_RELU_GN)) {
     if (plain && (!need_gn || table_ok)) {
-      hipLaunchKernelGGL((conv_split_kernel<BM, BN, PRO, NS, need_gn, false, false, true>), grid, dim3(256), 0, s, a);
+      if (close)
+        hipLaunchKernelGGL((conv_split_kernel<BM, BN, PRO, NS, need_gn, false, false, true, true>), grid, dim3(256), 0, s, a);
+      else
+        hipLaunchKernelGGL((conv_split_kernel<BM, BN, PRO, NS, need_gn, false, false, true>), grid, dim3(256), 0, s, a);
       SNAP_CHECK_LAUNCH();
       return a.ksplit > 1 ? launch_splitk_reduce(a, s) : SNAP_OK;
     }
   }
-  if (need_gn && table_ok)
+  if (close) {
+    if (need_gn && table_ok)
+      hipLaunchKernelGGL((conv_split_kernel<BM, BN, PRO, NS, need_gn, false, false, false, true>), grid, dim3(256), 0, s, a);
+    else
+      hipLaunchKernelGGL((conv_split_kernel<BM, BN, PRO, NS, false, false, false, false, true>), grid, dim3(256), 0, s, a);
+  } else if (need_gn && table_ok)
     hipLaunchKernelGGL((conv_split_kernel<BM, BN, PRO, NS, need_gn, false>), grid, dim3(256), 0, s, a);
   else if (tail)
     hipLaunchKernelGGL((conv_split_kernel<BM, BN, PRO, NS, false, true>), grid, dim3(256), 0, s, a);
diff --git a/snap_amd/ops.py b/snap_amd/ops.py
--- a/snap_amd/ops.py
+++ b/snap_amd/ops.py
@@ -38,6 +38,8 @@
     'CONV_RS_FORCE': False,
     'CONV_NO_WS': False,
     'SPLITK_STATS': True,
+    'SPLITK_CLOSE_IN_KERNEL': True,
+    'CONV_SPLITK': 0,
     'CONV_NO_PLAIN': False,
     'USE_PRESPLIT_VOTING': True,
     'PS_RES_INIT': True,
@@ -438,6 +440,8 @@
   ps_res_init: int
   bk_hint: int
   tune_flags: int
+  splitk_close: bool = False
+  counter_bytes: int = 0
 
 
 def plan_conv(
@@ -542,13 +546,17 @@
                      'no row lists)')
   kind = lib.snap_conv2d_stationary_kind(dref, qparts) if (qparts == 2 and no_rows) else 0
   pst = (T.PS_TILE if ps_tile is None else int(ps_tile)) if (ps or ps1) else 0
-  wbytes = sbytes = scount = rows32 = tile_rows = 0
-  gnb = False
+  wbytes = sbytes = scount = rows32 = tile_rows = force_s = 0
+  gnb = splitk_close = False
   if no_rows:
     if ps:
       wbytes = lib.snap_conv2d_presplit_workspace_bytes(dref, pst) if T.USE_SPLITK else 0
     elif not (ps1 or kind or out_half):
       wbytes = lib.snap_conv2d_workspace_bytes(dref) if T.USE_SPLITK else 0
+    force_s = int(T.CONV_SPLITK or 0) if (qparts >= 2 and not ps) else 0
+    if wbytes and force_s > 1:
+      wbytes = max(wbytes, force_s * M * Cout * 4)
+    splitk_close = bool(wbytes and qparts >= 2 and not ps and T.SPLITK_CLOSE_IN_KERNEL)
     if wbytes:
       half_engine = math in HALF_MATH and packed and Cin % 4 == 0 and not ps
       if emit_gn_stats is not None and (qparts >= 2 or half_engine) and T.SPLITK_STATS:
@@ -584,11 +592,12 @@
     if ps:
       xpre, res0 = 1, int(T.PS_RES_INIT if res_init is None else bool(res_init))
   bk_hint = tune_flags = 0
-  tuned = bool(T.CONV_BK or T.CONV_NO_HALO or T.CONV_RS_NSPLIT or T.CONV_NO_PLAIN)
+  tuned = bool(T.CONV_BK or T.CONV_NO_HALO or T.CONV_RS_NSPLIT or T.CONV_NO_PLAIN or force_s > 1)
   if tuned:
     bk_hint = int(T.CONV_BK or 0)
     tune_flags = (_lib.SNAP_TUNE_NO_HALO * int(bool(T.CONV_NO_HALO)) | _lib.SNAP_TUNE_NO_PLAIN * int(bool(T.CONV_NO_PLAIN))
-                  | ((int(T.CONV_RS_NSPLIT) & 15) << _lib.SNAP_TUNE_RS_NSPLIT_SHIFT))
+                  | ((int(T.CONV_RS_NSPLIT) & 15) << _lib.SNAP_TUNE_RS_NSPLIT_SHIFT)
+                  | (((force_s if force_s > 1 else 0) & 15) << _lib.SNAP_TUNE_SPLITK_SHIFT))
   return ConvPlan(
       desc=d, out_shape=(N, Ho, Wo, Cout), out_dtype=out_dtype, engine=math if image else 'f32', family=family,
       tag='PS_' if ps else 'PS1_' if ps1 else ('', 'RS_', 'WS_', 'WS_')[kind], image=image, parts=iparts,
@@ -596,7 +605,25 @@
       stats_bytes=sbytes, stats_count=scount, stats_relu=bool(sbytes) and emit_gn_stats == 'relu',
       gn_partial_rows=rows32, tile_rows=tile_rows, gnb=gnb,
       w_split_parts=iparts, w_split_root=root, w_half=int(image == 'fp16'), x_half=int(xh and not ps1),
-      x_presplit=xpre, ps_tile=pst if xpre else 0, ps_res_init=res0, bk_hint=bk_hint, tune_flags=tune_flags)
+      x_presplit=xpre, ps_tile=pst if xpre else 0, ps_res_init=res0, bk_hint=bk_hint, tune_flags=tune_flags,
+      splitk_close=splitk_close, counter_bytes=_lib.SNAP_SPLITK_COUNTER_BYTES if splitk_close else 0)
+
+
+_SPLITK_ARENAS = {}
+
+
+def _splitk_arena(dev, nbytes):
+  stream = _raw_stream(_raw_device()) if (_raw_stream is not None and _raw_device is not None) else \
+      torch.cuda.current_stream().cuda_stream
+  key = (dev.index, stream)
+  arena = _SPLITK_ARENAS.get(key)
+  if arena is None or arena.numel() * 4 < nbytes:
+    arena = torch.empty((nbytes + 3) // 4, dtype=torch.int32, device=dev)
+    arena[:_lib.SNAP_SPLITK_COUNTER_BYTES // 4].zero_()
+    arena._snap_stream = stream
+    _SPLITK_ARENAS[key] = arena
+  assert arena._snap_stream == stream and arena.device == dev, 'split-K arena: one per stream'
+  return arena
 
 
 def conv2d(
@@ -636,7 +663,10 @@
                 gn_bwd_stats, bf16_ring)
   dev = xd.device
   y = out if out is not None else torch.empty(p.out_shape, dtype=p.out_dtype, device=dev)
-  kws = torch.empty(p.workspace_bytes // 4, dtype=torch.float32, device=dev) if p.workspace_bytes else None
+  if p.splitk_close:
+    kws = _splitk_arena(dev, p.counter_bytes + p.workspace_bytes)
+  else:
+    kws = torch.empty(p.workspace_bytes // 4, dtype=torch.float32, device=dev) if p.workspace_bytes else None
   partial = torch.empty(p.stats_bytes // 4, dtype=torch.float32, device=dev) if p.stats_count else None
   partial2 = torch.empty(p.stats_bytes // 4, dtype=torch.float32, device=dev) if p.stats_count == 2 else None
   wpk = None
@@ -648,7 +678,7 @@
     if rows_in is not None or rows_out is not None or row_count is not None:
       ex.rows_in, ex.rows_out, ex.row_count = _pv(rows_in), _pv(rows_out), _pv(row_count)
     if kws is not None:
-      ex.workspace, ex.workspace_bytes = kws.data_ptr(), p.workspace_bytes
+      ex.workspace, ex.workspace_bytes = kws.data_ptr(), p.counter_bytes + p.workspace_bytes
     if partial is not None:
       ex.gn_partial, ex.gn_partial_bytes = partial.data_ptr(), p.stats_bytes
       ex.gn_partial_relu, ex.gn_partial_rows = int(p.stats_relu), p.gn_partial_rows
@@ -665,7 +695,7 @@
       ex.x_presplit, ex.ps_tile, ex.ps_res_init = p.x_presplit, p.ps_tile, p.ps_res_init
       if out_half:
         ex.y_half = y.data_ptr()
-    ex.bk_hint, ex.tune_flags = p.bk_hint, p.tune_flags
+    ex.bk_hint, ex.tune_flags = p.bk_hint, p.tune_flags | (_lib.SNAP_TUNE_SPLITK_CLOSE if p.splitk_close else 0)
   N, Ho, Wo, Cout = p.out_shape
   KH, KW, Cin = w.shape[:3]
   M = N * Ho * Wo
```

New measurement: 337.4 scenes/s. 0.828x the previous value.
